# KangWelly/Assignment-for-AAE6102_GNSS-SDR

Hardware: AMD Instinct MI355X
Metric: correlator Msamples/s (acq+track), whole job (higher is better)
Workload: dtype int8 in; acquisition: f64 correlation + f64 fine search; tracking: f64

## Files before the change

assignment-for-aae6102_gnss-sdr_amd/abi.py:

```python
from __future__ import annotations

import ctypes as C
import os
import sys

MAX_SV = 64
MAX_TAPS = 32

OK, ENODATA, EIO, EARG, EDEVICE, EINDEX = 0, 1, 2, 3, 4, 5

FIELDS = ["P_i", "P_q", "E_i", "E_q", "L_i", "L_q", "PLLdiscri", "DLLdiscri", "codedelay",
          "remChip", "codeFreq", "carrierFreq", "remPhase", "remSample", "numSample",
          "delayValue", "absoluteSample", "codedelay2"]
NFIELDS = len(FIELDS)
OUT_DEVICE = 1
FIELDS_POS = ["P_i", "P_q", "E_i", "E_q", "L_i", "L_q", "carrError", "codeError", "codedelay",
              "remChip", "codeFreq", "carrFreq", "remCarrPhase", "absoluteSampleCodedelay",
              "numSample", "delayValue", "absoluteSample", "codedelay2"]

MC_TAPS = 25
MC_TAP_NAMES = ([f"E_{{}}{s}" for s in ["_060", "_055", "", "_045", "_040", "_035", "_030", "_025",
                                         "_020", "_015", "_010", "_005"]] + ["P_{}"] +
                [f"L_{{}}{s}" for s in ["005", "010", "015", "020", "025", "030", "035", "040", "045",
                                         "", "055", "060"]])
# ... 143 lines not shown
    "gnss_abi_version": (C.c_int, []),
    "gnss_strerror": (C.c_char_p, [C.c_int]),
    "gnss_ctx_create": (C.c_int, [C.c_int, C.POINTER(C.c_void_p)]),
    "gnss_ctx_create_multi": (C.c_int, [C.POINTER(C.c_int), C.c_int, C.POINTER(C.c_void_p)]),
    "gnss_ctx_members": (C.c_int, [C.c_void_p]),
    "gnss_ctx_drop_record": (C.c_int, [C.c_void_p, C.c_void_p]),
    "gnss_ctx_resident_records": (C.c_int, [C.c_void_p]),
    "gnss_device_count": (C.c_int, []),
    "gnss_ctx_destroy": (None, [C.c_void_p]),
    "gnss_last_error": (C.c_char_p, [C.c_void_p]),
    "gnss_last_timing": (C.c_int, [C.c_void_p, C.POINTER(GnssTiming)]),
    "gnss_ctx_set_profiling": (C.c_int, [C.c_void_p, C.c_int]),
    "gnss_ctx_set_acq_precision": (C.c_int, [C.c_void_p, C.c_int]),
    "gnss_ctx_set_window": (C.c_int, [C.c_void_p, C.c_uint64]),
    "gnss_ctx_set_option": (C.c_int, [C.c_void_p, C.c_int, C.c_int64]),
    "gnss_dev_alloc": (C.c_int, [C.c_void_p, C.c_uint64, C.POINTER(C.c_void_p)]),
    "gnss_dev_free": (C.c_int, [C.c_void_p, C.c_void_p]),
    "gnss_dev_upload": (C.c_int, [C.c_void_p, C.c_void_p, C.c_void_p, C.c_uint64]),
    "gnss_dev_download": (C.c_int, [C.c_void_p, C.c_void_p, C.c_void_p, C.c_uint64]),
    "gnss_acquisition": (C.c_int, [C.c_void_p, C.POINTER(GnssFile), C.POINTER(GnssSignal),
                                   C.POINTER(GnssAcq), C.POINTER(GnssAcquired),
                                   C.POINTER(GnssAcqDiag)]),
    "gnss_tracking_ct": (C.c_int, [C.c_void_p, C.POINTER(GnssFile), C.POINTER(GnssSignal),
                                   C.POINTER(GnssTrack), C.POINTER(GnssAcquired),
                                   C.POINTER(GnssTrackOut)]),
    "gnss_tracking_ct_pos": (C.c_int, [C.c_void_p, C.POINTER(GnssFile), C.POINTER(GnssSignal),
                                       C.POINTER(GnssTrack), C.POINTER(GnssAcquired), C.c_int32,
                                       C.POINTER(C.c_int32), C.POINTER(GnssTrackOut)]),
    "gnss_tracking_ct_mc": (C.c_int, [C.c_void_p, C.POINTER(GnssFile), C.POINTER(GnssSignal),
                                      C.POINTER(GnssTrack), C.POINTER(GnssAcquired), C.c_int32,
                                      C.c_int32, C.POINTER(GnssTrackOut)]),
    "gnss_tracking_ct_multicorr": (C.c_int, [C.c_void_p, C.POINTER(GnssFile), C.POINTER(GnssSignal),
                                             C.POINTER(GnssTrack), C.POINTER(GnssAcquired), C.c_int32,
                                             C.POINTER(GnssTrackOut)]),
    "gnss_navi_decode": (C.c_int, [C.POINTER(GnssAcquired), C.POINTER(C.c_double),
                                   C.POINTER(C.c_int64), C.c_int64, C.POINTER(GnssNavOut)]),
    "gnss_lnav_bits": (C.c_int, [C.c_int32, C.c_int32, C.c_void_p]),
    "gnss_ca_code": (C.c_int, [C.c_int, C.c_void_p]),
    "gnss_correlate_step": (C.c_int, [C.c_void_p, C.POINTER(GnssFile), C.POINTER(GnssSignal),
                                      C.c_int, C.c_int, C.c_double, C.c_double, C.c_double,
                                      C.c_double, C.c_int64, C.c_int, C.POINTER(C.c_double),
                                      C.POINTER(C.c_double), C.POINTER(C.c_int64)]),
    "gnss_synth_if_device": (C.c_int, [C.c_void_p, C.POINTER(GnssSynth), C.c_uint64, C.c_uint64,
                                       C.c_void_p]),
    "gnss_tracking_vt_run": (C.c_int, [C.c_void_p, C.POINTER(GnssFile), C.POINTER(GnssSignal),
                                       C.POINTER(GnssTrack), C.c_int32, C.c_int32, C.c_int32,
                                       C.POINTER(GnssVtChan), C.POINTER(C.c_double), C.POINTER(GnssVtOut)]),
    "gnss_tracking_vt_step": (C.c_int, [C.c_void_p, C.POINTER(GnssFile), C.POINTER(GnssSignal),
                                        C.POINTER(GnssTrack), C.c_int32, C.c_int32, C.POINTER(GnssVtChan),
                                        C.POINTER(C.c_double), C.POINTER(GnssVtOut)]),
    "gnss_vt_nco_step": (C.c_int, [C.POINTER(GnssSignal), C.POINTER(GnssTrack), C.c_int32,
                                   C.POINTER(GnssVtChan), C.c_double, C.c_double, C.c_double,
                                   C.POINTER(GnssVtOut)]),
    "gnss_vt_prepare": (C.c_int, [C.POINTER(GnssSignal), C.c_int32, C.POINTER(GnssVtChan), C.c_double,
                                  C.POINTER(C.c_int32), C.POINTER(C.c_int64)]),
    "gnss_sv_pos_vel": (C.c_int, [C.POINTER(GnssEphSv), C.c_double, C.POINTER(C.c_double),
                                  C.POINTER(C.c_double), C.POINTER(C.c_double), C.POINTER(C.c_double),
                                  C.POINTER(C.c_double)]),
    "gnss_geo": (C.c_int, [C.c_int, C.POINTER(C.c_double), C.POINTER(C.c_double)]),
    "gnss_vt_nav_init": (C.c_int, [C.POINTER(GnssVtNavCfg), C.POINTER(GnssSignal), C.c_int32, C.c_int32,
                                   C.POINTER(C.c_int32), C.POINTER(GnssEphSv), C.POINTER(C.c_double),
                                   C.POINTER(C.c_double), C.c_double, C.c_double, C.POINTER(C.c_double),
                                   C.POINTER(GnssVtNav)]),
    "gnss_vt_nav_predict": (C.c_int, [C.POINTER(GnssVtNav), C.c_int32, C.c_int64, C.POINTER(C.c_double),
                                      C.POINTER(C.c_double), C.POINTER(C.c_double)]),
    "gnss_vt_nav_update": (C.c_int, [C.POINTER(GnssVtNav), C.POINTER(C.c_double), C.POINTER(C.c_double),
                                     C.POINTER(C.c_double), C.POINTER(GnssVtNavSol)]),
    "gnss_tracking_vt": (C.c_int, [C.c_void_p, C.POINTER(GnssFile), C.POINTER(GnssSignal), C.POINTER(GnssTrack),
                                   C.c_int32, C.c_int32, C.POINTER(GnssVtChan), C.POINTER(GnssVtNav),
                                   C.POINTER(GnssVtOut), C.POINTER(GnssVtNavSol)]),
    "gnss_tracking_vt_mc_run": (C.c_int, [C.c_void_p, C.POINTER(GnssFile), C.POINTER(GnssSignal),
                                          C.POINTER(GnssTrack), C.c_int32, C.c_int32, C.c_int32,
                                          C.POINTER(GnssVtChan), C.POINTER(C.c_double), C.POINTER(GnssVtMcOut)]),
    "gnss_tracking_vt_mc": (C.c_int, [C.c_void_p, C.POINTER(GnssFile), C.POINTER(GnssSignal), C.POINTER(GnssTrack),
                                      C.c_int32, C.c_int32, C.POINTER(GnssVtChan), C.POINTER(GnssVtNav),
                                      C.POINTER(GnssVtMcOut), C.POINTER(GnssVtNavSol)]),
    "gnss_vt_mc_prepare": (C.c_int, [C.POINTER(GnssSignal), C.c_int32, C.POINTER(GnssVtChan), C.c_double,
                                     C.POINTER(C.c_double), C.POINTER(C.c_double), C.POINTER(C.c_int64)]),
    "gnss_vt_mc_nco_step": (C.c_int, [C.POINTER(GnssSignal), C.POINTER(GnssTrack), C.c_int32,
                                      C.POINTER(GnssVtChan), C.c_double, C.POINTER(C.c_double),
                                      C.POINTER(C.c_double), C.POINTER(GnssVtMcOut)]),
    "gnss_vt_mc_nav_update": (C.c_int, [C.POINTER(GnssVtNav), C.POINTER(C.c_double), C.POINTER(C.c_double),
                                        C.POINTER(C.c_double), C.POINTER(GnssVtNavSol)]),
}

LIB_PATH = os.path.join(os.path.dirname(os.path.abspath(__file__)), "lib", "libgnss_mi355x.so")
_lib = None
_torch_first = False
LOADED_PATH = None

(OPT_FORCE_SUB, OPT_NO_PERSIST, OPT_FORCE_VPB, OPT_ACQ_ROCFFT, OPT_FINE_ROCFFT, OPT_ACQ_BATCH, OPT_ACQ_FUSED,
 OPT_ACQ_RING, OPT_ACQ_PIPE, OPT_VT_BLOCKS, OPT_FORCE_PEER, OPT_VT_SPAN) = range(12)
MAX_DEVICES = 16


def require_torch():
    import torch
    if _lib is not None and not _torch_first:
        raise RuntimeError("import torch before the first gnss Context / abi.load() "
                           "(PyTorch-ROCm must bring up its HIP runtime first)")
    return torch


class GnssError(RuntimeError):
    def __init__(self, status, msg=""):
        self.status = status
        super().__init__(f"gnss status {status}: {msg}")


def load(path: str | None = None):
    global _lib
    if _lib is not None and path is None:
        return _lib
    p = path or os.environ.get("GNSS_LIB") or LIB_PATH
    if not os.path.exists(p):
        raise ImportError(f"{p} missing: the HIP extension is not built "
                          "(run `python -c 'import __graft_entry__ as g; g.build()'`)")
    global _torch_first
    if _lib is None:
        if "torch" not in sys.modules and os.environ.get("GNSS_NO_TORCH", "0") != "1":
            try:
                import torch
            except Exception:
                pass
        _torch_first = "torch" in sys.modules
    lib = C.CDLL(p)
    for name, (res, args) in PROTOTYPES.items():
        if p != LIB_PATH and not hasattr(lib, name):
            continue
        fn = getattr(lib, name)
        fn.restype = res
        fn.argtypes = args
    if path is None:
        global LOADED_PATH
        _lib = lib
        LOADED_PATH = os.path.abspath(p)
    return lib
```

assignment-for-aae6102_gnss-sdr_amd/csrc/gnss_api.cpp:

```cpp
#include <hip/hip_runtime.h>
#include <rocfft/rocfft.h>

#include <algorithm>
#include <chrono>
#include <cstdarg>
#include <cmath>
#include <cstdio>
#include <cstring>
#include <cstdlib>
#include <functional>
#include <thread>
#include <vector>
#include <fcntl.h>
#include <map>
#include <memory>
#include <mutex>
#include <string>
#include <tuple>
#include <unistd.h>
#include <vector>

#include "gnss_internal.h"
#include "group.h"
#include "vt_mc.h"

using namespace gnss;

struct gnss_ctx {
    int device = 0;
    hipStream_t stream = nullptr;
    hipStream_t stream2 = nullptr;
    hipEvent_t ev_cols[2] = {}, ev_rows[2] = {};
    std::string err;
    gnss_timing timing{};
    int profiling = 0;
    std::map<std::tuple<size_t, size_t, int, int>, rocfft_plan> plans;
    void* fft_work = nullptr;
    size_t fft_work_size = 0;
    std::map<std::string, std::pair<void*, size_t>> pool;
    std::map<std::string, std::pair<void*, size_t>> pinned;
    int64_t acq_tw_S = 0;
    int acq_tw_dbl = -1;
    int acq_fp64 = 1;
    uint64_t window = 0;
    int64_t opt[GNSS_OPT_COUNT] = {};
    std::vector<gnss_ctx*> members;
    bool member = false;
    int fail_chan = -1;
    gnss::group::ResidentCache<void*> resident;
};

static void release_resident(void* p)
{
    if (p) (void)hipFree(p);
}

static int drop_resident(gnss_ctx* ctx, const void* p, uint64_t n)
{
    int k = 0;
    for (gnss_ctx* m : ctx->members) {
        (void)hipSetDevice(m->device);
        if (m->stream) (void)hipStreamSynchronize(m->stream);
        if (!p) {
            k += (int)m->resident.m.size();
            m->resident.clear(release_resident);
        } else {
            k += m->resident.drop_overlapping(p, n, release_resident);
        }
    }
    (void)hipSetDevice(ctx->device);
    return k;
}

#ifndef GNSS_PROBE_BUILD
#define GNSS_PROBE_BUILD 0
#endif
static const char* probe_env(const char* name)
{
    return GNSS_PROBE_BUILD ? getenv(name) : nullptr;
}

namespace {
constexpr int kAcqPipeDefault = 2;
#ifndef GNSS_ACQ_FWD_SPLIT
#define GNSS_ACQ_FWD_SPLIT 1
#endif
constexpr bool kAcqFwdSplit = GNSS_ACQ_FWD_SPLIT;
constexpr int kAcqPairFront = 60;
constexpr int kVtSpan = 2000;
constexpr int kFineBatch = 16;

template <class T>
T* pinned_buffer(gnss_ctx* ctx, const char* key, size_t count, unsigned flags = hipHostMallocDefault)
{
    auto& e = ctx->pinned[key];
    const size_t want = std::max<size_t>(count * sizeof(T), 16);
    if (e.second < want) {
        if (e.first) (void)hipHostFree(e.first);
        e = {nullptr, 0};
        if (hipHostMalloc(&e.first, want, flags) != hipSuccess) return nullptr;
        e.second = want;
    }
    return static_cast<T*>(e.first);
}
}

namespace {

int fail(gnss_ctx* ctx, int code, const char* fmt, ...) __attribute__((format(printf, 3, 4)));
int fail(gnss_ctx* ctx, int code, const char* fmt, ...)
{
    char buf[512];
    va_list ap;
    va_start(ap, fmt);
    vsnprintf(buf, sizeof buf, fmt, ap);
    va_end(ap);
    if (ctx) ctx->err = buf;
    return code;
}

bool lane_rate_admitted(const gnss_signal* sg, double codeFreq_max)
{
    return sg->Fs > 0 && 8.0 * std::max(sg->codeFreqBasis * 1.01, codeFreq_max) / sg->Fs < 1.0;
}

int refuse_lane_rate(gnss_ctx* ctx, const gnss_signal* sg, double codeFreq_max)
{
    return fail(ctx, GNSS_EARG,
// ... 697 lines not shown
    }
    std::vector<int> ds(devices, devices + n);
    std::sort(ds.begin(), ds.end());
    ds.erase(std::unique(ds.begin(), ds.end()), ds.end());
    for (int a : ds)
        for (int b : ds) {
            int can = 0;
            if (a == b || hipDeviceCanAccessPeer(&can, a, b) != hipSuccess || !can) continue;
            if (hipSetDevice(a) == hipSuccess) (void)hipDeviceEnablePeerAccess(b, 0);
            (void)hipGetLastError();
        }
    (void)hipSetDevice(devices[0]);
    *out = g;
    return GNSS_OK;
}

int gnss_device_count(void)
{
    int n = 0;
    if (hipGetDeviceCount(&n) != hipSuccess) return 0;
    return n;
}

int gnss_ctx_members(const gnss_ctx* ctx)
{
    if (!ctx) return 0;
    return ctx->members.empty() ? 1 : (int)ctx->members.size();
}

void gnss_ctx_destroy(gnss_ctx* ctx)
{
    if (!ctx) return;
    for (gnss_ctx* m : ctx->members) gnss_ctx_destroy(m);
    ctx->members.clear();
    (void)hipSetDevice(ctx->device);
    if (ctx->stream) (void)hipStreamSynchronize(ctx->stream);
    ctx->resident.clear(release_resident);
    if (ctx->stream2) (void)hipStreamSynchronize(ctx->stream2);
    for (auto& kv : ctx->plans) rocfft_plan_destroy(kv.second);
    if (ctx->fft_work) (void)hipFree(ctx->fft_work);
    for (auto& kv : ctx->pool)
        if (kv.second.first) (void)hipFree(kv.second.first);
    for (auto& kv : ctx->pinned)
        if (kv.second.first) (void)hipHostFree(kv.second.first);
    for (int i = 0; i < 2; i++) {
        if (ctx->ev_cols[i]) (void)hipEventDestroy(ctx->ev_cols[i]);
        if (ctx->ev_rows[i]) (void)hipEventDestroy(ctx->ev_rows[i]);
    }
    if (ctx->stream2) (void)hipStreamDestroy(ctx->stream2);
    if (ctx->stream) (void)hipStreamDestroy(ctx->stream);
    delete ctx;
}

const char* gnss_last_error(const gnss_ctx* ctx) { return ctx ? ctx->err.c_str() : "no context"; }

int gnss_last_timing(const gnss_ctx* ctx, gnss_timing* out)
{
    if (!ctx || !out) return GNSS_EARG;
    *out = ctx->timing;
    return GNSS_OK;
}

int gnss_ctx_set_profiling(gnss_ctx* ctx, int enable)
{
    if (!ctx) return GNSS_EARG;
    ctx->profiling = enable;
    for (gnss_ctx* m : ctx->members) m->profiling = enable;
    return GNSS_OK;
}

int gnss_ctx_set_window(gnss_ctx* ctx, uint64_t bytes)
{
    if (!ctx) return GNSS_EARG;
    ctx->window = bytes;
    for (gnss_ctx* m : ctx->members) m->window = bytes;
    return GNSS_OK;
}

int gnss_ctx_set_option(gnss_ctx* ctx, int key, int64_t value)
{
    if (!ctx || key < 0 || key >= GNSS_OPT_COUNT) return GNSS_EARG;
    if (key == GNSS_OPT_VT_BLOCKS && (value < 0 || value > GNSS_VT_MAX_BLOCKS))
        return fail(ctx, GNSS_EARG, "GNSS_OPT_VT_BLOCKS outside 0..%d", GNSS_VT_MAX_BLOCKS);
    if (key == GNSS_OPT_VT_SPAN && (value < 0 || value > kVtSpan))
        return fail(ctx, GNSS_EARG, "GNSS_OPT_VT_SPAN outside 0..%d", kVtSpan);
    ctx->opt[key] = value;
    for (gnss_ctx* m : ctx->members) m->opt[key] = value;
    return GNSS_OK;
}

int gnss_ctx_set_acq_precision(gnss_ctx* ctx, int fp64)
{
    if (!ctx || (fp64 != 0 && fp64 != 1)) return GNSS_EARG;
    ctx->acq_fp64 = fp64;
    for (gnss_ctx* m : ctx->members) m->acq_fp64 = fp64;
    return GNSS_OK;
}

int gnss_dev_alloc(gnss_ctx* ctx, uint64_t nbytes, void** dev_ptr)
{
    if (!ctx || !dev_ptr) return GNSS_EARG;
    HIP_TRY(hipSetDevice(ctx->device));
    HIP_TRY(hipMalloc(dev_ptr, nbytes ? nbytes : 16));
    return GNSS_OK;
}

int gnss_ctx_drop_record(gnss_ctx* ctx, const void* dev_ptr)
{
    if (!ctx) return GNSS_EARG;
    drop_resident(ctx, dev_ptr, 0);
    return GNSS_OK;
}

int gnss_ctx_resident_records(const gnss_ctx* ctx)
{
    if (!ctx) return 0;
    int k = 0;
    for (const gnss_ctx* m : ctx->members) k += (int)m->resident.m.size();
    return k;
}

int gnss_dev_free(gnss_ctx* ctx, void* p)
{
    if (!ctx) return GNSS_EARG;
    drop_resident(ctx, p, 0);
    HIP_TRY(hipSetDevice(ctx->device));
    HIP_TRY(hipFree(p));
    return GNSS_OK;
}

int gnss_dev_upload(gnss_ctx* ctx, void* dst, const void* src, uint64_t n)
{
    if (!ctx) return GNSS_EARG;
    drop_resident(ctx, dst, n);
    HIP_TRY(hipSetDevice(ctx->device));
    HIP_TRY(hipMemcpyAsync(dst, src, n, hipMemcpyHostToDevice, ctx->stream));
    HIP_TRY(hipStreamSynchronize(ctx->stream));
    return GNSS_OK;
}

int gnss_dev_download(gnss_ctx* ctx, void* dst, const void* src, uint64_t n)
{
    if (!ctx) return GNSS_EARG;
    HIP_TRY(hipSetDevice(ctx->device));
    HIP_TRY(hipMemcpyAsync(dst, src, n, hipMemcpyDeviceToHost, ctx->stream));
    HIP_TRY(hipStreamSynchronize(ctx->stream));
    return GNSS_OK;
}

int gnss_acquisition(gnss_ctx* ctx, const gnss_file* file, const gnss_signal* sg,
                     const gnss_acq* acq, gnss_acquired* out, gnss_acq_diag* diag)
{
    if (!ctx || !file || !sg || !acq || !out) return GNSS_EARG;
    if (!ctx->members.empty()) return group_acquisition(ctx, file, sg, acq, out, diag);
    memset(out, 0, sizeof(*out));
    if (diag) memset(diag, 0, sizeof(*diag));
    ctx->timing = gnss_timing{};
    HIP_TRY(hipSetDevice(ctx->device));
    const int prec = file->dataPrecision, dtyp = file->dataType;
    if ((prec != 1 && prec != 2) || (dtyp != 1 && dtyp != 2))
        return fail(ctx, GNSS_EARG, "dataPrecision must be 1 (int8) or 2 (int16), dataType 1 (I) or 2 (I/Q)");
    if (prec == 2 && dtyp == 1)
        return fail(ctx, GNSS_EINDEX, "int16 real record: rawsignal has Sample*datalen/2 samples (MATLAB index error)");
    const int64_t bps = (int64_t)prec * dtyp;
    const bool iq8 = prec == 1 && dtyp == 2;
    const int64_t S = sg->Sample;
// ... 329 lines not shown
        }
        const int64_t c0 = (S - cd + 1 + (file->skip + N1 + 18) * S) * bps;
        const int64_t a1 = (S - cd + 1 + file->skip * S) * bps + (int64_t)((N1 + 18) * S * 1.01 + 64) * bps;
        hi = std::max(hi, std::max(c0 + (int64_t)(n10 * 10 * S * 1.01 + 4096) * bps, a1));
        hiA = std::max(hiA, a1);
    }
    P.file_len = file_length(file);
    if (P.file_len < 0) return fail(ctx, GNSS_EIO, "cannot open IF record");
    IfWindow w;
    lo &= ~(int64_t)31;
    const bool seg = ctx->window > 0 && !file->dev_data && !pos && !gv && prec == 1 && dtyp == 2 && n10 > 0 &&
                     (uint64_t)(hi - lo) > ctx->window;
    int st;
    if (seg) {
        if ((uint64_t)(hiA - lo) > ctx->window || ctx->window < (uint64_t)(12 * S * bps * 1.01 + 8192))
            return fail(ctx, GNSS_EARG, "window budget below the 1-ms phases' span");
        HIP_TRY(w.own.alloc(ctx->window + 64));
        w.ptr = w.own.as<int8_t>();
        w.base = lo;
        w.len = std::min<int64_t>(hiA, P.file_len) - lo;
        if ((st = stage_into(ctx, file, w.base, w.base + w.len, w.own.as<int8_t>()))) return st;
    } else if ((st = stage_window(ctx, file, lo, hi, w))) {
        return st;
    }
    const int8_t* iq_dev = w.ptr;
    P.buf_base = w.base;
    P.buf_len = w.len;
    DevBuf d_conv, d_pref, d_pscr;
    {
        const int64_t s0 = std::max<int64_t>(lo, w.base);
        const int64_t s1 = std::min<int64_t>(hi, w.base + w.len);
        const int8_t* src = w.ptr + (s0 - w.base);
        if (prec == 1 && dtyp == 1) {
            const int64_t n = std::max<int64_t>(s1 - s0, 0);
            HIP_TRY(d_conv.alloc(ctx, "trk.d_conv", (size_t)(2 * n + 64)));
            HIP_TRY(launch_real8_to_iq8(src, n, d_conv.as<int8_t>(), ctx->stream));
            iq_dev = d_conv.as<int8_t>();
            P.buf_base = 2 * s0;
            P.buf_len = 2 * n;
        } else if (prec == 2) {
            iq_dev = src;
            P.buf_base = s0;
            P.buf_len = std::max<int64_t>(s1 - s0, 0);
            const int64_t ng = P.buf_len / 32;
            HIP_TRY(d_pref.alloc(ctx, "trk.d_pref", 2 * sizeof(long long) * (size_t)(ng + 1)));
            const size_t scr = prefix16_scratch_bytes(ng);
            HIP_TRY(d_pscr.alloc(ctx, "trk.d_pscr", scr));
            long long* pi = d_pref.as<long long>();
            HIP_TRY(launch_prefix16(reinterpret_cast<const short*>(src), ng, pi, pi + ng + 1, d_pscr.p, scr,
                                    ctx->stream));
            P.pref_i = pi;
            P.pref_q = pi + ng + 1;
            P.stage16 = reinterpret_cast<const short*>(iq_dev - P.buf_base);
        }
    }

    const double cps_max = 1.1 * sg->codeFreqBasis / sg->Fs;
    auto sub_ok = [&](int sub) { return 8.0 * sub * cps_max < 1.0 && (sub == 1 || !P.exact_div); };
    auto sub_for = [&](int pdi) {
        int sub = pdi >= 10 ? 3 : 1;
        while (sub > 1 && !sub_ok(sub)) sub--;
        if ((P.fmt == 1 || ntaps == 25) && sub != 3) sub = 1;
        return sub;
    };
    int sub1 = sub_for(1), sub10 = sub_for(10);
    if (const char* fs = probe_env("GNSS_FORCE_SUB10")) {
        const int v = atoi(fs);
        if (v >= 1 && v <= 4 && sub_ok(v) && P.fmt == 0 && ntaps != 25) sub10 = v;
    }
    if (const char* fs = probe_env("GNSS_FORCE_SUB1")) {
        const int v = atoi(fs);
        if (v >= 1 && v <= 4 && sub_ok(v) && P.fmt == 0 && ntaps != 25) sub1 = v;
    }
    if (const int v = (int)ctx->opt[GNSS_OPT_FORCE_SUB]) {
        if (v >= 1 && v <= 4 && sub_ok(v) && ((P.fmt == 0 && ntaps != 25) || v == 1 || v == 3)) sub1 = sub10 = v;
    }
    auto bpc_for = [&](int pdi, int sub) {
        const double groups = (S * pdi * 1.01 + 64) / 8.0 + 2;
        return (int)std::ceil(groups / ((double)kTrkThreads * sub));
    };
    int cus = 0;
    HIP_TRY(hipDeviceGetAttribute(&cus, hipDeviceAttributeMultiprocessorCount, ctx->device));
    P.qcap_dmax = cps_max;
    auto qcap_ok = [&](int sub) {
        return !GNSS_QCAP || P.ntaps <= 3 ||
               max_taps_in_lane(P.taps, P.tap_post, P.ntaps, 8 * sub, cps_max) <= kQcapMax;
    };
    auto vpb_for = [&](int pdi, int sub) {
        if (ctx->opt[GNSS_OPT_NO_PERSIST] || P.fmt != 0 || wide_taps || bpc_for(pdi, sub) > run_bpc_cap(P.ntaps) ||
            !qcap_ok(sub))
            return 0;
        const int bpc = bpc_for(pdi, sub);
        int v0 = 1;
        if (ctx->opt[GNSS_OPT_FORCE_VPB] > 0) v0 = (int)std::min<int64_t>(ctx->opt[GNSS_OPT_FORCE_VPB], kMaxVpb);
        const int occ1 = std::min(track_run_blocks_per_cu(P, sub, false), 4);
        if (v0 == 1 && occ1 >= 1 && (int64_t)nch * bpc <= (int64_t)occ1 * cus) return 1;
        const int occv = std::min(track_run_blocks_per_cu(P, sub, true), 4);
        if (occv < 1) return 0;
        for (int v = std::max(v0, 2); v <= kMaxVpb; v++)
            if ((int64_t)nch * ((bpc + v - 1) / v) <= (int64_t)occv * cus) return v;
        return 0;
    };
    const int vpb1 = vpb_for(1, sub1), vpb10 = vpb_for(10, sub10);
    bool persist1 = vpb1 > 0, persist10 = vpb10 > 0;
    if (const char* pr = probe_env("GNSS_PROBE")) P.probe = atoi(pr);
    const int bpc1 = bpc_for(1, sub1), bpc10 = bpc_for(10, sub10);
    if (bpc10 > kMaxBpc) return fail(ctx, GNSS_EARG, "Sample too large for the step geometry");

    std::vector<TrkChan> ch0((size_t)nch);
    std::vector<unsigned> cab((size_t)nch * 32);
    for (int i = 0; i < nch; i++) {
        const int c = chans[i];
        TrkChan& t = ch0[i];
        memset(&t, 0, sizeof(t));
        t.codeFreq = sg->codeFreqBasis;
        t.carrierFreqBasis = acq->fineFreq[c];
        t.carrierFreq = acq->fineFreq[c];
        t.codedelay0 = acq->codedelay[c];
        t.pos = (S - acq->codedelay[c] + 1 + file->skip * S) * bps;
        t.snrIndex = 1;
        t.sv1 = c + 1;
        t.prn = acq->sv[c];
        t.n1_target = N1;
        if (pos) {
            t.pos = (int64_t)(((double)S - acq->codedelay[c] + 1 + (double)file->skip * sg->Fs * sg->ms) * bps);
            t.codedelay0 = S - acq->codedelay[c] + 1;
            t.sv1 = 1;
            t.n1_target = pos_n1(c);
            t.countinx = pos->countinx ? pos->countinx[c] : 0;
        }
        if (gv) t.pos = (S - acq->codedelay[c] - 1 + file->skip * S) * bps;
        if (acq->sv[c] < 1 || acq->sv[c] > 51) return fail(ctx, GNSS_EARG, "bad PRN");
        ca_bits(acq->sv[c], &cab[(size_t)i * 32]);
    }
    DevBuf d_chan, d_snap, d_desc, d_ca, d_part, d_arrive, d_rec, d_taps, d_cn1, d_cn10, d_dv, d_pi;
    HIP_TRY(d_chan.alloc(ctx, "trk.d_chan", sizeof(TrkChan) * nch));
    HIP_TRY(d_snap.alloc(ctx, "trk.d_snap", sizeof(TrkChan) * nch));
    HIP_TRY(d_desc.alloc(ctx, "trk.d_desc", sizeof(StepDesc) * nch));
    HIP_TRY(d_ca.alloc(ctx, "trk.d_ca", sizeof(unsigned) * cab.size()));
    HIP_TRY(d_part.alloc(ctx, "trk.d_part", sizeof(double) * (size_t)nch * kMaxBpc * 2 * ntaps));
    const size_t arrive_bytes = sizeof(unsigned) * kArrivePerChan * kArriveStride * nch;
    HIP_TRY(d_arrive.alloc(ctx, "trk.d_arrive", arrive_bytes));
    HIP_TRY(d_rec.alloc(ctx, "trk.d_rec", sizeof(double) * (size_t)nch * P.rec_cap * GNSS_NFIELDS));
    if (out->taps) HIP_TRY(d_taps.alloc(ctx, "trk.d_taps", sizeof(double) * (size_t)nch * P.rec_cap * 2 * ntaps));
    HIP_TRY(d_cn1.alloc(ctx, "trk.d_cn1", sizeof(double) * (size_t)nch * P.cn0_cap));
    HIP_TRY(d_cn10.alloc(ctx, "trk.d_cn10", sizeof(double) * (size_t)nch * P.cn0_cap));
    HIP_TRY(d_dv.alloc(ctx, "trk.d_dv", sizeof(int64_t) * (size_t)nch * (P.rec_cap + 1)));
    HIP_TRY(d_pi.alloc(ctx, "trk.d_pi", sizeof(double) * (size_t)nch * N1));
    HIP_TRY(hipMemcpyAsync(d_chan.p, ch0.data(), sizeof(TrkChan) * nch, hipMemcpyHostToDevice, ctx->stream));
    HIP_TRY(hipMemcpyAsync(d_ca.p, cab.data(), sizeof(unsigned) * cab.size(), hipMemcpyHostToDevice, ctx->stream));
    HIP_TRY(hipMemsetAsync(d_arrive.p, 0, arrive_bytes, ctx->stream));
    HIP_TRY(hipMemsetAsync(d_cn1.p, 0, d_cn1.n, ctx->stream));
    HIP_TRY(hipMemsetAsync(d_cn10.p, 0, d_cn10.n, ctx->stream));
    HIP_TRY(hipMemsetAsync(d_dv.p, 0, d_dv.n, ctx->stream));
    HIP_TRY(hipMemsetAsync(d_rec.p, 0, d_rec.n, ctx->stream));

    TrkBuffers B{};
    B.iq = iq_dev;
    B.chan = d_chan.as<TrkChan>();
    B.snap = d_snap.as<TrkChan>();
    B.desc = d_desc.as<StepDesc>();
    B.ca_bits = d_ca.as<unsigned>();
    B.partial = d_part.as<double>();
    B.arrive = d_arrive.as<unsigned>();
    B.rec = d_rec.as<double>();
    B.taps_rec = out->taps ? d_taps.as<double>() : nullptr;
    B.cn0_1 = d_cn1.as<double>();
    B.cn0_10 = d_cn10.as<double>();
    B.dvpre = d_dv.as<int64_t>();
    B.p_i_1ms = d_pi.as<double>();
    B.n1 = N1;

    DevBuf d_stamps;
    const char* stamp_path = probe_env("GNSS_STAMPS");
    if (stamp_path) {
        HIP_TRY(d_stamps.alloc(ctx, "trk.d_stamps", sizeof(unsigned long long) * ((size_t)kStampSlots * (8 + 3 * kMaxBpc) + 1)));
        HIP_TRY(hipMemsetAsync(d_stamps.p, 0, d_stamps.n, ctx->stream));
        B.stamps = d_stamps.as<unsigned long long>();
    }

    DevBuf d_pgran, d_err;
    if (persist1 || persist10) {
        HIP_TRY(d_pgran.alloc(ctx, "trk.d_pgran", sizeof(unsigned long long) * 2 * (size_t)nch * gran_per_chan(ntaps)));
        HIP_TRY(d_err.alloc(ctx, "trk.d_err", 16));
        HIP_TRY(hipMemsetAsync(d_pgran.p, 0, d_pgran.n, ctx->stream));
        HIP_TRY(hipMemsetAsync(d_err.p, 0, 16, ctx->stream));
        B.pgran = d_pgran.as<unsigned long long>();
        B.run_err = d_err.as<unsigned>();
    }
// ... 253 lines not shown
        const double* src;
        int64_t stride;
        if (f < nrf) {
            dst = out->rec + ((int64_t)c * GNSS_NFIELDS + f) * ML;
            src = rec + (size_t)i * P.rec_cap * GNSS_NFIELDS + f;
            stride = GNSS_NFIELDS;
        } else {
            const int tq = f - nrf, sidx = tq / 2, iq = tq % 2;
            dst = out->taps + (((int64_t)c * 2 + iq) * ntaps + sidx) * ML;
            src = tp + (size_t)i * P.rec_cap * 2 * ntaps + tq;
            stride = 2 * ntaps;
        }
        for (int64_t k = 0; k < n1; k++) dst[k] = src[k * stride];
        for (int64_t q = 0; q < n10; q++) {
            const double v = src[(n1 + q) * stride];
            for (int r = 0; r < 10; r++) dst[n1 + 10 * q + r] = v;
        }
        for (int64_t k = n1 + 10 * n10; k < ML; k++) dst[k] = 0;
    });
    if (hp) fprintf(stderr, "hostprof expanded %.3f ms\n", hms());
    if (gv && out->rec) {
        for (int c = 0; c < nsv; c++) {
            double* cdr = out->rec + ((int64_t)c * GNSS_NFIELDS + GNSS_F_codedelay) * ML;
            double sum = 0;
            for (int64_t k = 0; k < N1; k++) {
                const int r = (int)(k % nsv);
                if (r <= c) sum += out->rec[((int64_t)r * GNSS_NFIELDS + GNSS_F_delayValue) * ML + k / nsv];
                cdr[k] = (double)acq->codedelay[c] + sum;
            }
        }
    }
    rows = std::max(rows, n10 / 20);
    out->cn0_rows = rows;
    if (out->CN0_Eph) {
        for (int i = 0; i < nch; i++) {
            const int c = chans[i];
            const int cx = chh[i].countinx;
            const int r1 = pos ? rows : std::max(N1, N1 + cx) / 20, r10 = n10 / 20;
            for (int r = 0; r < out->cn0_cap; r++) {
                double v = 0;
                if (r < r10) v = cn10[(size_t)i * P.cn0_cap + r];
                else if (r < r1) v = cn1[(size_t)i * P.cn0_cap + r];
                out->CN0_Eph[(int64_t)r * nsv + c] = v;
            }
        }
    }
    return GNSS_OK;
}

int gnss_tracking_ct(gnss_ctx* ctx, const gnss_file* file, const gnss_signal* sg, const gnss_track* tr,
                     const gnss_acquired* acq, gnss_track_out* out)
{
    if (ctx && !ctx->members.empty()) return group_tracking(ctx, file, sg, tr, acq, out, nullptr);
    return tracking_impl(ctx, file, sg, tr, acq, out, nullptr);
}

int gnss_tracking_ct_pos(gnss_ctx* ctx, const gnss_file* file, const gnss_signal* sg, const gnss_track* tr,
                         const gnss_acquired* acq, int32_t ctPOS, const int32_t* countinx, gnss_track_out* out)
{
    const PosCfg pc{ctPOS, countinx, 0};
    if (ctx && !ctx->members.empty()) return group_tracking(ctx, file, sg, tr, acq, out, &pc);
    return tracking_impl(ctx, file, sg, tr, acq, out, &pc);
}

int gnss_tracking_ct_multicorr(gnss_ctx* ctx, const gnss_file* file, const gnss_signal* sg,
                               const gnss_track* tr, const gnss_acquired* acq, int32_t datalength,
                               gnss_track_out* out)
{
    const GivenCfg g{datalength};
    return tracking_impl(ctx, file, sg, tr, acq, out, nullptr, &g);
}

int gnss_tracking_ct_mc(gnss_ctx* ctx, const gnss_file* file, const gnss_signal* sg, const gnss_track* tr,
                        const gnss_acquired* acq, int32_t msPosCT, int32_t pdi, gnss_track_out* out)
{
    if (!ctx) return GNSS_EARG;
    if (pdi != 1 && pdi != 10) return fail(ctx, GNSS_EARG, "multicorrelator: pdi must be 1 or 10");
    if (msPosCT < pdi) return fail(ctx, GNSS_EARG, "multicorrelator: msPosCT/pdi must be >= 1");
    const PosCfg pc{msPosCT / pdi, nullptr, pdi};
    if (!ctx->members.empty()) return group_tracking(ctx, file, sg, tr, acq, out, &pc);
    return tracking_impl(ctx, file, sg, tr, acq, out, &pc);
}

int gnss_correlate_step(gnss_ctx* ctx, const gnss_file* file, const gnss_signal* sg, int prn, int pdi,
                        double remChip, double codeFreq, double carrierFreq, double remPhase,
                        int64_t pos_bytes, int n_taps, const double* taps, double* sums_out,
                        int64_t* numSample_out)
{
    if (!ctx || !file || !sg || !taps || !sums_out || (n_taps != 3 && n_taps != 11) || prn < 1 || prn > 51)
        return GNSS_EARG;
    if (pdi != 1 && pdi != 10) return GNSS_EARG;
    if (!lane_rate_admitted(sg, codeFreq)) return refuse_lane_rate(ctx, sg, codeFreq);
    HIP_TRY(hipSetDevice(ctx->device));
    const int64_t S = sg->Sample;
    TrkParams P{};
    P.Fs = sg->Fs;
    P.codeFreqBasis = sg->codeFreqBasis;
    P.ms = sg->ms;
    P.codelength = sg->codelength;
    P.S = (double)S;
    P.dataBytesPerSample = 2;
    P.bps = 2;
    P.fmt = 0;
    P.inv_Fs = 1.0 / sg->Fs;
    P.exact_div = fast_div_exact(sg->Fs, (int64_t)(S * 10 * 1.02) + 64) ? 0 : 1;
    P.ntaps = n_taps;
    P.iE = 0; P.iP = n_taps / 2; P.iL = n_taps - 1;
    for (int s = 0; s < n_taps; s++) P.taps[s] = taps[s];
    P.nsv = P.nch = 1;
    P.rec_cap = 1;
    P.cn0_cap = 1;
    P.file_len = file_length(file);
    IfWindow w;
    int st = stage_window(ctx, file, pos_bytes, pos_bytes + (int64_t)(2.1 * S * pdi) + 64, w);
    if (st) return st;
    P.buf_base = w.base;
    P.buf_len = w.len;
    TrkChan c{};
    c.remChip = remChip;
    c.codeFreq = codeFreq;
    c.carrierFreq = carrierFreq;
    c.remPhase = remPhase;
    c.pos = pos_bytes;
    c.n1_target = 1 << 30;
    c.sv1 = 1;
    c.prn = prn;
    unsigned cab[32];
    ca_bits(prn, cab);
    int sub = 1;
    if (const int v = (int)ctx->opt[GNSS_OPT_FORCE_SUB]) {
        if (v >= 2 && v <= 4 && !P.exact_div && 8.0 * v * codeFreq / sg->Fs < 1.0) sub = v;
    }
    const int bpc = (int)std::ceil(((S * pdi * 1.01 + 64) / 8.0 + 2) / ((double)kTrkThreads * sub));
    DevBuf d_chan, d_desc, d_ca, d_part, d_arrive, d_sums;
    HIP_TRY(d_chan.alloc(sizeof(TrkChan)));
    HIP_TRY(d_desc.alloc(sizeof(StepDesc)));
    HIP_TRY(d_ca.alloc(sizeof(cab)));
    HIP_TRY(d_part.alloc(sizeof(double) * kMaxBpc * 2 * n_taps));
    HIP_TRY(d_arrive.alloc(sizeof(unsigned) * kArrivePerChan * kArriveStride));
    HIP_TRY(d_sums.alloc(sizeof(double) * 2 * n_taps));
    HIP_TRY(hipMemcpyAsync(d_chan.p, &c, sizeof c, hipMemcpyHostToDevice, ctx->stream));
    HIP_TRY(hipMemcpyAsync(d_ca.p, cab, sizeof cab, hipMemcpyHostToDevice, ctx->stream));
    HIP_TRY(hipMemsetAsync(d_arrive.p, 0, sizeof(unsigned) * kArrivePerChan * kArriveStride, ctx->stream));
    TrkBuffers B{};
    B.iq = w.ptr;
    B.chan = d_chan.as<TrkChan>();
    B.desc = d_desc.as<StepDesc>();
    B.ca_bits = d_ca.as<unsigned>();
    B.partial = d_part.as<double>();
    B.arrive = d_arrive.as<unsigned>();
    B.dbg_sums = d_sums.as<double>();
    DevBuf d_args;
    HIP_TRY(d_args.alloc(sizeof(TrkParams) + sizeof(TrkBuffers)));
    HIP_TRY(hipMemcpyAsync(d_args.p, &P, sizeof(TrkParams), hipMemcpyHostToDevice, ctx->stream));
    HIP_TRY(hipMemcpyAsync(static_cast<char*>(d_args.p) + sizeof(TrkParams), &B, sizeof(TrkBuffers),
                           hipMemcpyHostToDevice, ctx->stream));
    const TrkDev TD{d_args.as<TrkParams>(),
                    reinterpret_cast<const TrkBuffers*>(static_cast<char*>(d_args.p) + sizeof(TrkParams))};

    HIP_TRY(launch_track_prepare(P, B, TD, pdi, 0, ctx->stream));
    HIP_TRY(launch_track_step(P, B, TD, bpc, sub, ctx->stream));
    HIP_TRY(hipMemcpyAsync(sums_out, d_sums.p, sizeof(double) * 2 * n_taps, hipMemcpyDeviceToHost, ctx->stream));
    HIP_TRY(hipMemcpyAsync(&c, d_chan.p, sizeof c, hipMemcpyDeviceToHost, ctx->stream));
    HIP_TRY(hipStreamSynchronize(ctx->stream));
    if (c.status) return fail(ctx, c.status, "correlate step failed");
    if (numSample_out) {
        const double cps = codeFreq / sg->Fs;
        *numSample_out = (int64_t)round((sg->codelength * pdi - remChip) / cps);
    }
    return GNSS_OK;
}

}

void gnss::ca_chips(int prn, float* out) { generate_ca(prn, out); }

extern "C" {

int gnss_tracking_vt_run(gnss_ctx* ctx, const gnss_file* file, const gnss_signal* sg, const gnss_track* tr,
                         int32_t pdi, int32_t n, int32_t nsteps, gnss_vt_chan* chans, const double* codeFreq_new,
                         gnss_vt_out* out)
{
    if (!ctx || !file || !sg || !tr || !chans || !codeFreq_new || !out || n < 1 || n > GNSS_MAX_SV || pdi < 1 ||
        nsteps < 1 || !(sg->Fs > 0) || !(sg->codeFreqBasis > 0))
        return fail(ctx, GNSS_EARG, "bad arguments");
    ctx->err.clear();
    ctx->timing = gnss_timing{};
    HIP_TRY(hipSetDevice(ctx->device));
    const int prec = file->dataPrecision, dtyp = file->dataType;
    if (!((prec == 1 && (dtyp == 1 || dtyp == 2)) || (prec == 2 && dtyp == 2)))
        return fail(ctx, GNSS_EARG, "vector tracking: int8 I/Q, int8 real or int16 I/Q records");
    const int bps = prec * dtyp;
    const int64_t flen = file_length(file);
    if (flen < 0) return fail(ctx, GNSS_EIO, "cannot open IF record");
    double cf_min = 1e300;
    for (int i = 0; i < n; i++) {
        if (chans[i].prn < 1 || chans[i].prn > 51) return fail(ctx, GNSS_EARG, "bad PRN");
        if (chans[i].file_ptr < 0 || chans[i].file_ptr % bps) return fail(ctx, GNSS_EARG, "file_ptr");
        if (chans[i].index_int < 0 || chans[i].index_int > 19 || chans[i].snrIndex < 1)
            return fail(ctx, GNSS_EARG, "C/N0 state (index_int 0..19, snrIndex >= 1)");
        cf_min = std::min(cf_min, chans[i].codeFreq);
    }
    for (int64_t k = 0; k < (int64_t)nsteps * n; k++) cf_min = std::min(cf_min, codeFreq_new[k]);
    if (!(cf_min > 0)) return fail(ctx, GNSS_EARG, "code frequencies must be positive");
    const double nmax = std::ceil((sg->codelength * pdi + 2.0) / (cf_min / sg->Fs)) + 2;
    int64_t lo = INT64_MAX, hi = 0;
    for (int i = 0; i < n; i++) {
        lo = std::min(lo, chans[i].file_ptr);
        hi = std::max(hi, chans[i].file_ptr + (int64_t)(nsteps * nmax) * bps);
    }
    IfWindow w;
    int st = stage_window(ctx, file, lo, std::min(hi, flen), w);
    if (st) return st;
    std::vector<unsigned> cab((size_t)n * 32);
    for (int i = 0; i < n; i++) ca_bits(chans[i].prn, &cab[(size_t)i * 32]);
// ... 770 lines not shown
```

assignment-for-aae6102_gnss-sdr_amd/csrc/gnss_internal.h:

```cpp
#pragma once

#include <hip/hip_runtime.h>
#include <stdint.h>

#include "../../include/gnss_mi355x.h"

#define GNSS_HD __host__ __device__ __forceinline__

namespace gnss {

struct Colon {
    double a, d, c;
    int64_t n;
};

GNSS_HD Colon colon_make(double a, double d, double b)
{
    Colon r{a, d, b, -1};
    if (!(a - a == 0) || !(d - d == 0) || !(b - b == 0)) return r;
    if (d == 0 || (a < b && d < 0) || (b < a && d > 0)) return r;
    double tol = 2.0 * 2.220446049250313e-16 * fmax(fabs(a), fabs(b));
    double sig = d > 0 ? 1.0 : -1.0;
    double n;
    if (a == floor(a) && d == 1) {
// ... 125 lines not shown
    const int n = (int)q & 3;
    const double a = (n & 1) ? c : s, b = (n & 1) ? s : c;
    *sn = (n & 2) ? -a : a;
    *cs = ((n + 1) & 2) ? -b : b;
}


typedef unsigned u32x4 __attribute__((ext_vector_type(4)));
constexpr int kBufRsrcWord3 = 0x00020000;
constexpr int kPolSc1 = 16;

__device__ __forceinline__ void publish16(__amdgpu_buffer_rsrc_t r, int unit, double v, unsigned tag)
{
    const unsigned long long w = (unsigned long long)__double_as_longlong(v);
    const u32x4 g = {(unsigned)w, tag, (unsigned)(w >> 32), tag};
    __builtin_amdgcn_raw_buffer_store_b128(g, r, unit * 16, 0, kPolSc1);
}
__device__ __forceinline__ u32x4 load16(__amdgpu_buffer_rsrc_t r, int unit)
{
    return __builtin_amdgcn_raw_buffer_load_b128(r, unit * 16, 0, kPolSc1);
}
constexpr int kPolSys = 17;
__device__ __forceinline__ void publish16_sys(__amdgpu_buffer_rsrc_t r, int unit, double v, unsigned tag)
{
    const unsigned long long w = (unsigned long long)__double_as_longlong(v);
    const u32x4 g = {(unsigned)w, tag, (unsigned)(w >> 32), tag};
    __builtin_amdgcn_raw_buffer_store_b128(g, r, unit * 16, 0, kPolSys);
}
__device__ __forceinline__ u32x4 load16_sys(__amdgpu_buffer_rsrc_t r, int unit)
{
    return __builtin_amdgcn_raw_buffer_load_b128(r, unit * 16, 0, kPolSys);
}
__device__ __forceinline__ double value16(u32x4 g)
{
    return __longlong_as_double((long long)(((unsigned long long)g.z << 32) | g.x));
}

struct TrkChan {
    double remChip, remPhase, remSample;
    double carrier_outputLast, PLLdiscriLast, code_outputLast, DLLdiscriLast;
    double codeFreq, carrierFreqBasis, carrierFreq;
    double Zk[20];
    int64_t numSample;
    int64_t pos;
    int64_t Index;
    int64_t nstep;
    int64_t slot;
    int64_t n1_target;
    int64_t codedelay0;
    int32_t index_int, snrIndex;
    int32_t sv1;
    int32_t prn;
    int32_t status;
    int32_t countinx;
};

struct TrkParams {
    double Fs, codeFreqBasis, ms, codelength;
    double S;
    double tau1code, tau2code, tau1carr, tau2carr;
    double dataBytesPerSample;
    double inv_Fs;
    int32_t exact_div;
    int64_t buf_base;
    int64_t buf_len;
    int64_t file_len;
    int32_t ntaps, iE, iP, iL;
    int32_t nsv;
    int32_t nch;
    int32_t rec_cap;
    int32_t cn0_cap;
    int32_t probe;
    int32_t bps, fmt;
    const long long* pref_i;
    const long long* pref_q;
    const short* stage16;
    double taps[GNSS_MAX_TAPS];
    double qcap_dmax;
    double dll_r, dll_t1, dll_t10, pll_r, pll_t1, pll_t10;
    int32_t conv;
    int32_t chip_off;
    int32_t given;
    double tap_post[GNSS_MAX_TAPS];
};

constexpr int kLaneMax = 32;

struct StepDesc {
    int64_t n, delayValue, A, g_first, g_last, Index;
    double remSample, d, inv_d, f, phi0, dhi, dlo, remChip_next, remPhase_next;
    double mu_r, mu_i;
    double phi[kLaneMax];
    double2 rcs[kLaneMax];
    double tap_a[GNSS_MAX_TAPS], tap_c[GNSS_MAX_TAPS];
    double rc0;
    int32_t pdi, phaseC;
    int32_t bad;
    int32_t bad_tap;
};

struct TrkBuffers {
    const int8_t* iq;
    TrkChan* chan;
    TrkChan* snap;
    StepDesc* desc;
    const unsigned* ca_bits;
    double* partial;
    unsigned int* arrive;
    double* rec;
    double* taps_rec;
    double* cn0_1;
    double* cn0_10;
    int64_t* dvpre;
    double* p_i_1ms;
    double* dbg_sums;
    unsigned long long* stamps;
    unsigned long long* pgran;
    unsigned* run_err;
    int32_t n1;
};

struct TrkDev {
    const TrkParams* p;
    const TrkBuffers* b;
};

hipError_t launch_track_step(const TrkParams& p, const TrkBuffers& b, const TrkDev& d,
                             int blocks_per_chan, int sub, hipStream_t s);
hipError_t launch_track_run(const TrkParams& p, const TrkBuffers& b, const TrkDev& d,
                            int blocks_per_chan, int vblocks_per_block, int sub, int nsteps, unsigned tag0,
                            hipStream_t s);
int track_run_blocks_per_cu(const TrkParams& p, int sub, bool vblocks = false);
hipError_t launch_track_prepare(const TrkParams& p, const TrkBuffers& b, const TrkDev& d, int pdi,
                                int phaseC, hipStream_t s);
hipError_t launch_track_snapshot(const TrkParams& p, const TrkBuffers& b, const TrkDev& d, hipStream_t s);
hipError_t launch_track_bitedge(const TrkParams& p, const TrkBuffers& b, const TrkDev& d, hipStream_t s);
hipError_t launch_track_phase_c_init(const TrkParams& p, const TrkBuffers& b, const TrkDev& d,
                                     int64_t skip, hipStream_t s);
hipError_t launch_track_expand(const double* src, int64_t rec_cap, int stride, int nf, int nch,
                               const int64_t* job, double* dst, int64_t ML, int64_t n10, int ntaps,
                               hipStream_t s);

#ifndef GNSS_PROBE_BUILD
#define GNSS_PROBE_BUILD 0
#endif
constexpr bool kProbe = GNSS_PROBE_BUILD != 0;
#ifndef GNSS_XCHG_SLEEP
#define GNSS_XCHG_SLEEP 0
#endif
#ifndef GNSS_XCD_LOCAL
#define GNSS_XCD_LOCAL 0
#endif

constexpr int kTrkThreads = 256;
constexpr int kArriveStride = 64;
constexpr int kArrivePerChan = 9;
constexpr int kStampSlots = 2200;
constexpr int kMaxBpc = 1024;
constexpr int kMaxBpcRun = 256;
constexpr int run_bpc_cap(int ntaps) { return ntaps > 3 ? 192 : kMaxBpcRun; }
constexpr int kMaxVpb = 16;
#ifndef GNSS_QCAP
#define GNSS_QCAP 0
#endif
constexpr double kTapSpan = 30.0;
constexpr int kQcapMax = 8;

inline int max_taps_in_lane(const double* taps, const double* post, int n, int M, double dmax)
{
    const double w = (M - 1) * dmax + 1e-9;
    int best = 0;
    for (int a = 0; a < n; a++) {
        const double x = taps[a] + (post ? post[a] : 0.0);
        int c = 0;
        for (int b = 0; b < n; b++) {
            double f = (taps[b] + (post ? post[b] : 0.0)) - x;
            f -= floor(f);
            if (f < w || f > 1.0 - 1e-9) c++;
        }
        best = c > best ? c : best;
    }
    return best;
}
constexpr int kDeferSlots = 4;
constexpr int gran_region_b(int ntaps) { return ntaps > 3 ? 2 * kMaxBpcRun * 6 : 0; }
constexpr int gran_slot_b(int ntaps) { return 2 * ntaps * kMaxBpcRun; }
constexpr int gran_per_chan(int ntaps)
{
    return ntaps > 3 ? gran_region_b(ntaps) + kDeferSlots * gran_slot_b(ntaps) : 2 * kMaxBpcRun * 2 * ntaps;
}
constexpr int kDescWords = (int)(sizeof(StepDesc) / 4);

struct AcqPeak {
    double peak;
    int32_t fbin;
    int32_t cp;
    double snr;
    double peak2;
};

hipError_t launch_acq_wipe(const int8_t* iq, const double2* xs, int64_t S, int datalen, int nbins, double IF,
                           double freqMin, double freqStep, double Fs, float2* out, hipStream_t s);
hipError_t launch_acq_code(const float* ca, const int32_t* prn_slot, int nprn, int64_t S,
                           double codeFreqBasis, double Fs, float2* out, hipStream_t s);
hipError_t launch_acq_mul(const float2* code_spec, const float2* sig_spec, int nprn, int nsig,
                          int64_t S, float2* out, hipStream_t s);
hipError_t launch_acq_power(const float2* y, int nprn, int nbins, int datalen, int64_t S,
                            int first_ms, float* corr, hipStream_t s);
hipError_t launch_acq_wipe(const int8_t* iq, const double2* xs, int64_t S, int datalen, int nbins, double IF,
                           double freqMin, double freqStep, double Fs, double2* out, hipStream_t s);
hipError_t launch_acq_code(const float* ca, const int32_t* prn_slot, int nprn, int64_t S,
                           double codeFreqBasis, double Fs, double2* out, hipStream_t s);
hipError_t launch_acq_mul(const double2* code_spec, const double2* sig_spec, int nprn, int nsig,
                          int64_t S, double2* out, hipStream_t s);
hipError_t launch_acq_power(const double2* y, int nprn, int nbins, int datalen, int64_t S,
                            int first_ms, double* corr, hipStream_t s);
hipError_t launch_acq_peak(const float* corr, int nprn, int nbins, int64_t S, int cshift,
                           int perm, AcqPeak* out, void* scratch, hipStream_t s);
hipError_t launch_acq_peak(const double* corr, int nprn, int nbins, int64_t S, int cshift,
                           int perm, AcqPeak* out, void* scratch, hipStream_t s);

bool acq_fft_supported(int64_t S);
template <class V>
hipError_t launch_acq_fft_forward(const int8_t* iq, const double2* xs, int64_t S, int datalen, int nbins, double IF,
                                  double freqMin, double freqStep, double Fs, const float* ca,
                                  int nprn, double codeFreqBasis, const V* tw_row,
                                  const V* tw_col, V* B, V* X, hipStream_t s, int bin0 = 0, int nbc = -1,
                                  bool codes = true);
constexpr int kAcqCols = 1, kAcqRows = 2;
hipError_t launch_acq_fft_correlate(const float2* C, const float2* X, int64_t S, int datalen,
                                    int nbins, int nprn, int first_pair, int npair,
                                    const float2* tw_row, const float2* tw_col, float2* A,
                                    float* corr, hipStream_t s, int parts = kAcqCols | kAcqRows);
hipError_t launch_acq_fft_correlate(const double2* C, const double2* X, int64_t S, int datalen,
                                    int nbins, int nprn, int first_pair, int npair,
                                    const double2* tw_row, const double2* tw_col, double2* A,
                                    double* corr, hipStream_t s, int parts = kAcqCols | kAcqRows);
hipError_t launch_acq_fft_pair(const double2* C, const double2* X, int64_t S, int datalen, int nbins, int nprn,
                               int cols_first, int cols_n, double2* Acols, int rows_first, int rows_n,
                               const double2* Arows, const double2* tw_row, const double2* tw_col, double* corr,
                               int front, hipStream_t s);
size_t acq_fused_sync_bytes();
size_t acq_fused_err_offset();
size_t acq_fused_ring_bytes(int64_t S);
hipError_t launch_acq_fft_correlate_fused(const double2* C, const double2* X, int64_t S, int datalen, int nbins,
                                          int nprn, int nslot, const double2* tw_row, const double2* tw_col,
                                          double2* ring, void* sync, double* corr, hipStream_t s);
bool fine_fft_supported(int64_t S, int L);
size_t fine_fft_scratch_bytes(int64_t S, int L, int datalen, int nsv);
hipError_t launch_fine_fft_tables(int64_t S, int L, int datalen, void* scratch, hipStream_t s);
hipError_t launch_fine_fft_argmax(const int8_t* iq, const double2* xs, int64_t S, int L, int datalen,
                                  const int32_t* cd, int nsv, const float* ca, double Fs, double codeFreqBasis,
                                  double codelength, int shifted, void* scratch, int64_t* kbest, hipStream_t s);
hipError_t launch_fine_build(const int8_t* iq, const double2* xs, int64_t S, int L, const int32_t* codedelay,
                             const float* ca, int nsv, double Fs, double codeFreqBasis,
                             double codelength, int64_t N, double2* out, hipStream_t s);
hipError_t launch_fine_argmax(const double2* F, int nsv, int64_t N, int shifted, void* scratch,
                              int64_t* kbest, hipStream_t s);

size_t acq_scratch_bytes(int nprn, int nsv);

hipError_t launch_stage_cpx(const int8_t* src, int prec, int type, int64_t nsamp, double2* out,
                            unsigned long long* sums, hipStream_t s);
hipError_t launch_real8_to_iq8(const int8_t* src, int64_t n, int8_t* dst, hipStream_t s);
size_t prefix16_scratch_bytes(int64_t ngroups);
// ... 268 lines not shown
```

assignment-for-aae6102_gnss-sdr_amd/csrc/track.hip:

```cpp
#include "gnss_internal.h"

namespace gnss {

namespace {

constexpr int kStampRow = 8 + 3 * kMaxBpc;

__device__ __forceinline__ unsigned long long* stamp_row(const TrkBuffers& b)
{
    const unsigned long long cnt = __hip_atomic_load(b.stamps + (size_t)kStampSlots * kStampRow,
                                                     __ATOMIC_RELAXED, __HIP_MEMORY_SCOPE_AGENT);
    return b.stamps + (cnt % kStampSlots) * kStampRow;
}

__device__ __forceinline__ void stamp_max(unsigned long long* row, int k, unsigned long long v)
{
    row[k] = v;
}

__device__ __forceinline__ int uni(int v) { return __builtin_amdgcn_readfirstlane(v); }
__device__ __forceinline__ int64_t uni(int64_t v)
{
    const int lo = __builtin_amdgcn_readfirstlane((int)v);
    const int hi = __builtin_amdgcn_readfirstlane((int)(v >> 32));
    return (int64_t)(((uint64_t)(uint32_t)hi << 32) | (uint32_t)lo);
}
__device__ __forceinline__ double uni(double v) { return __longlong_as_double(uni((int64_t)__double_as_longlong(v))); }

typedef int i32x4 __attribute__((ext_vector_type(4)));
typedef __attribute__((address_space(1))) const i32x4 g_i32x4;
typedef __attribute__((address_space(1))) double g_dbl;
typedef __attribute__((address_space(1))) long long g_i64;
typedef __attribute__((address_space(1))) unsigned g_u32;
typedef __attribute__((address_space(1))) unsigned long long g_u64;
typedef __attribute__((address_space(1))) const StepDesc g_desc;
typedef __attribute__((address_space(1))) const TrkChan g_chan;
typedef __attribute__((address_space(1))) const unsigned g_cu32;

__device__ __forceinline__ int4 ld_g16(const int8_t* p)
{
    const i32x4 v = *(g_i32x4*)p;
    return make_int4(v.x, v.y, v.z, v.w);
}

__device__ __forceinline__ double ld_sc1(const double* ptr)
{
    return __hip_atomic_load((g_dbl*)ptr, __ATOMIC_RELAXED, __HIP_MEMORY_SCOPE_AGENT);
}

__device__ __forceinline__ void st_sc1(double* ptr, double v)
{
    __hip_atomic_store((g_dbl*)ptr, v, __ATOMIC_RELAXED, __HIP_MEMORY_SCOPE_AGENT);
}

__device__ __forceinline__ unsigned atomic_add_agent(unsigned* p, unsigned v)
{
    return __hip_atomic_fetch_add((g_u32*)p, v, __ATOMIC_RELAXED, __HIP_MEMORY_SCOPE_AGENT);
}

__device__ __forceinline__ void store_agent(unsigned* p, unsigned v)
{
    __hip_atomic_store((g_u32*)p, v, __ATOMIC_RELAXED, __HIP_MEMORY_SCOPE_AGENT);
}

__device__ __forceinline__ void store_agent(unsigned long long* p, unsigned long long v)
{
    __hip_atomic_store((g_u64*)p, v, __ATOMIC_RELAXED, __HIP_MEMORY_SCOPE_AGENT);
}

__device__ __forceinline__ unsigned long long load_agent(const unsigned long long* p)
{
    return __hip_atomic_load((g_u64*)p, __ATOMIC_RELAXED, __HIP_MEMORY_SCOPE_AGENT);
}

struct TailK {
    double Fs, inv_Fs, codelength, S, codeFreqBasis, ms;
    double dll_r, dll_t1, dll_t10, pll_r, pll_t1, pll_t10, tau1code, tau1carr, qcap_dmax;
    int32_t exact_div, conv, given, chip_off, ntaps, iE, iP, iL, bps;
    int64_t file_len, buf_base, buf_len;
    const double* taps;
    const double* tap_post;
    static constexpr int fmt = 0;
    static constexpr const long long* pref_i = nullptr;
// ... 454 lines not shown
        index_int = 0;
        snrIndex += 1;
    }
    g->remChip = o.remChip;
    g->remPhase = o.remPhase;
    g->remSample = o.remSample;
    g->carrier_outputLast = u.carrier_output;
    g->PLLdiscriLast = u.PLLdiscri;
    g->code_outputLast = u.code_output;
    g->DLLdiscriLast = u.DLLdiscri;
    g->codeFreq = u.codeFreq;
    g->carrierFreq = u.carrierFreq;
    g->numSample = o.n;
    g->pos = c.pos + p.bps * o.n;
    g->Index = c.Index + (o.phaseC ? 10 : 1);
    g->nstep = c.nstep + 1;
    g->slot = c.slot + 1;
    g->index_int = index_int;
    g->snrIndex = snrIndex;
}
__device__ __noinline__ void write_state(const TrkParams& p, const TrkBuffers& b, int ch, TrkChan* g, const TrkChan& c, const StepOut& o, const LoopUpd& u, const double* s, bool io)
{
    write_state_i(p, b, ch, g, c, o, u, s, io);
}

__device__ __forceinline__ void update_state_inplace(const TrkParams& p, const TrkBuffers& b, int ch,
                                                     TrkChan& c, const StepOut& o, const LoopUpd& u,
                                                     const double* s, bool io)
{
    const double P_i = s[2 * p.iP], P_q = s[2 * p.iP + 1];
    int index_int = c.index_int + 1;
    int snrIndex = c.snrIndex;
    c.Zk[index_int - 1] = P_i * P_i + P_q * P_q;
    if (index_int % 20 == 0) {
        if (io) {
            double Z[20];
#pragma unroll
            for (int k = 0; k < 20; k++) Z[k] = c.Zk[k];
            const double cn = cn0_estimate(Z, 1 * p.ms * o.pdi);
            g_dbl* cn0 = (g_dbl*)(o.phaseC ? b.cn0_10 : b.cn0_1);
            if (snrIndex <= p.cn0_cap) cn0[(int64_t)ch * p.cn0_cap + snrIndex - 1] = cn;
        }
        index_int = 0;
        snrIndex += 1;
    }
    const int64_t pos = c.pos, Index = c.Index, nstep = c.nstep, slot = c.slot;
    c.remChip = o.remChip;
    c.remPhase = o.remPhase;
    c.remSample = o.remSample;
    c.carrier_outputLast = u.carrier_output;
    c.PLLdiscriLast = u.PLLdiscri;
    c.code_outputLast = u.code_output;
    c.DLLdiscriLast = u.DLLdiscri;
    c.codeFreq = u.codeFreq;
    c.carrierFreq = u.carrierFreq;
    c.numSample = o.n;
    c.pos = pos + p.bps * o.n;
    c.Index = Index + (o.phaseC ? 10 : 1);
    c.nstep = nstep + 1;
    c.slot = slot + 1;
    c.index_int = index_int;
    c.snrIndex = snrIndex;
}


}

__device__ __forceinline__ double2 ld_rcs(const StepDesc* d, int m) { return d->rcs[m]; }
__device__ __forceinline__ double2 ld_rcs(g_desc* d, int m)
{
    typedef __attribute__((address_space(1))) const double g_cdbl;
    g_cdbl* q = (g_cdbl*)&d->rcs[m];
    return make_double2(q[0], q[1]);
}

template <int SUB> struct RegRaw {
    const int4 (&r)[SUB];
    __device__ __forceinline__ int4 get(int j) const { return r[j]; }
};
struct LdsRaw {
    const int4* p;
    __device__ __forceinline__ int4 get(int j) const { return p[j * kTrkThreads]; }
};

#ifndef GNSS_CORR_PROBE
#define GNSS_CORR_PROBE 0
#endif
#ifndef GNSS_IO_DR_WAVE
#define GNSS_IO_DR_WAVE 2
#endif
#ifndef GNSS_SWEEP_IO_ALL
#define GNSS_SWEEP_IO_ALL 0
#endif
#ifndef GNSS_FLUSH_PROBE
#define GNSS_FLUSH_PROBE 0
#endif

__device__ __forceinline__ unsigned ca_bits_ext(unsigned cabits, int lane)
{
    const unsigned w0 = __shfl(cabits, 0, 64), w1 = __shfl(cabits, 1, 64), w2 = __shfl(cabits, 2, 64);
    if (lane == 31) return cabits | ((w0 & 1u) << 31);
    if (lane == 32) return (w0 >> 1) | (w1 << 31);
    if (lane == 33) return (w1 >> 1) | (w2 << 31);
    return cabits;
}

#ifndef GNSS_SWP
#define GNSS_SWP 0
#endif
#ifndef GNSS_REGCAP
#define GNSS_REGCAP 0
#endif
#ifndef GNSS_PHI_REG
#define GNSS_PHI_REG 0
#endif
#ifndef GNSS_TAPWIN
#define GNSS_TAPWIN 1
#endif
template <int NT, int SUB, bool DIVIDE, bool RELOAD, int FMT, class Desc, class Raw>
__device__ __forceinline__ void lane_correlate(const TrkParams& p, const Desc* dp, const Raw& raw,
                                               int64_t ks, unsigned cabits, double2* myslot,
                                               const double2* zero, double (&oI)[NT], double (&oQ)[NT],
                                               const double* posts = nullptr)
{
    constexpr int M = 8 * SUB;
    constexpr int T = kTrkThreads;
    constexpr bool QC = RELOAD && (GNSS_QCAP == 2 || (GNSS_QCAP && NT > 3));
    if constexpr ((GNSS_CORR_PROBE & 8) != 0) {
#pragma unroll
        for (int s = 0; s < NT; s++) { oI[s] = 0.0; oQ[s] = 0.0; }
        return;
    }
    const int64_t n = uni(dp->n);
    const double d = uni(dp->d), inv_d = uni(dp->inv_d);
    const double f = uni(dp->f), phi0 = uni(dp->phi0);
    const double Fs = p.Fs, rFs = p.inv_Fs;

    const int ksi = (int)ks, ni = (int)n;
    const int lo = ksi < 0 ? (-ksi < M ? -ksi : M) : 0;
    const int hi = ni - ksi < M ? (ni - ksi > 0 ? ni - ksi : 0) : M;

    const int kfi0 = ksi + lo;
    const int kfi = kfi0 < 0 ? 0 : (kfi0 > ni - 1 ? ni - 1 : kfi0);
    const int64_t kf = kfi;
    int cap[NT];
    unsigned neg0 = 0u, neg1 = 0u;
    constexpr bool TW = GNSS_TAPWIN && RELOAD && (GNSS_CORR_PROBE & 66) == 0;
    if constexpr (TW) {
        const int nn = ni - 1;
        const bool mid = 2 * kfi == nn, lower = kfi <= nn / 2;
        const double KD = (double)kfi * d, NKD = (double)(nn - kfi) * d;
        const double kend = lower ? KD : -NKD;
        const double dk = (double)(kfi - ksi);
        int c0i[NT];
        int cmin = 0x7fffffff;
        bool exact = mid;
#pragma unroll
        for (int s = 0; s < NT; s++) {
            const double a = lds_at(dp->tap_a, s), c = lds_at(dp->tap_c, s);
            const double t0 = ((lower ? a : c) + kend) + lds_at(posts, s);
            const double c0 = ceil(t0);
            const double R = __builtin_fma(c0 - t0, inv_d, dk);
            exact = exact || fabs(R - rint(R)) < 1e-6;
            const int pb = (int)floor(R) + 1;
            cap[s] = (pb < M ? pb : M) - 1;
            c0i[s] = (int)c0;
        }
        if (exact) {
#pragma unroll
            for (int s = 0; s < NT; s++) {
                const double a = lds_at(dp->tap_a, s), c = lds_at(dp->tap_c, s);
                const double post = lds_at(posts, s);
                const double t0 = (mid ? (a + c) / 2 : lower ? a + KD : c - NKD) + post;
                const double c0 = ceil(t0);
                const double R = dk + (c0 - t0) * inv_d;
                const double rr = rint(R);
                int pb = (int)floor(R) + 1;
                if (fabs(R - rr) < 1e-6) {
                    const int ms = (int)rr;
                    pb = ms;
                    const int64_t kx = ks + ms;
                    if (ms >= 0 && ms < M && kx >= 0 && kx <= n - 1)
                        pb = ceil(colon_elem(Colon{a, d, c, (int64_t)nn}, kx) + post) > c0 ? ms : ms + 1;
                }
                cap[s] = (pb < M ? pb : M) - 1;
                c0i[s] = (int)c0;
            }
        }
#pragma unroll
        for (int s = 0; s < NT; s++) {
            if constexpr ((GNSS_CORR_PROBE & 32) != 0) cap[s] = M - 1 - s;
            cmin = c0i[s] < cmin ? c0i[s] : cmin;
        }
        const unsigned ib = ca_index32(cmin + p.chip_off);
        const unsigned wlo = __shfl(cabits, (int)(ib >> 5), 64), whi = __shfl(cabits, (int)(ib >> 5) + 1, 64);
        const unsigned long long W = (((unsigned long long)whi << 32) | wlo) >> (ib & 31);
#pragma unroll
        for (int s = 0; s < NT; s++) {
            const int o = c0i[s] - cmin;
            neg0 |= (unsigned)((W >> o) & 1ull) << s;
            neg1 |= (unsigned)((W >> (o + 1)) & 1ull) << s;
        }
    }
#pragma unroll
    for (int s = 0; s < (TW ? 0 : NT); s++) {
        if constexpr ((GNSS_CORR_PROBE & 2) != 0) {
            cap[s] = M - 1 - s;
            neg0 |= (cabits & 1u) << s;
            continue;
        }
        if constexpr ((GNSS_CORR_PROBE & 64) != 0) {
            cap[s] = (int)((ks + 5 * s) & 31) - 4;
            neg0 |= (cabits & 1u) << s;
            continue;
        }
        const Colon col{uni(dp->tap_a[s]), d, uni(dp->tap_c[s]), n - 1};
        const double post = p.tap_post[s];
        const double t0 = colon_elem(col, kf) + post;
        const double c0 = ceil(t0);
        const double R = (double)(int)(kf - ks) + (c0 - t0) * inv_d;
        const double rr = rint(R);
        int pb = (int)floor(R) + 1;
        if (fabs(R - rr) < 1e-6) {
            const int ms = (int)rr;
            pb = ms;
            const int64_t kx = ks + ms;
            if (ms >= 0 && ms < M && kx >= 0 && kx <= n - 1)
                pb = ceil(colon_elem(col, kx) + post) > c0 ? ms : ms + 1;
        }
        cap[s] = (pb < M ? pb : M) - 1;
        if constexpr ((GNSS_CORR_PROBE & 32) != 0) cap[s] = M - 1 - s;
        const unsigned i0 = ca_index32((int)c0 + p.chip_off);
        const unsigned i1 = i0 == 1022u ? 0u : i0 + 1u;
        const unsigned w0 = __shfl(cabits, (int)(i0 >> 5), 64);
        const unsigned w1 = __shfl(cabits, (int)(i1 >> 5), 64);
        neg0 |= ((w0 >> (i0 & 31)) & 1u) << s;
        neg1 |= ((w1 >> (i1 & 31)) & 1u) << s;
    }

    const double kb = (double)(int)ks;
    const double Wb = wave_at<DIVIDE>(kb, f, phi0, Fs, rFs);
    double sb, cb;
    if constexpr ((GNSS_CORR_PROBE & 1) != 0) {
        sb = Wb * 1e-9;
        cb = 1.0;
    } else {
        sincos_wave(Wb, &sb, &cb);
    }

    double run_r = 0.0, run_i = 0.0;
    double pre_r[QC ? 1 : NT], pre_i[QC ? 1 : NT];
    if constexpr (!QC) {
#pragma unroll
        for (int s = 0; s < NT; s++) { pre_r[s] = 0.0; pre_i[s] = 0.0; }
    }
    unsigned cmask = 0u;
    if constexpr (QC) {
#pragma unroll
        for (int s = 0; s < NT; s++)
            if (cap[s] >= 0 && cap[s] < M - 1) cmask |= 1u << cap[s];
    }

    double mu_r = 0.0, mu_i = 0.0;
    if constexpr (FMT == 1) {
        mu_r = uni(dp->mu_r);
        mu_i = uni(dp->mu_i);
    }

    constexpr bool RC = GNSS_REGCAP && !QC && NT <= 3;
    double dhi_l = 0.0, dlo_l = 0.0;
    if constexpr (GNSS_PHI_REG) {
        dhi_l = uni(dp->dhi);
        dlo_l = uni(dp->dlo);
    }
    double Wpipe = 0.0;
    if constexpr (GNSS_SWP) Wpipe = wave_at<DIVIDE>(kb + 1.0, f, phi0, Fs, rFs);
    auto subgroup = [&](const int j) {
        constexpr int NW = FMT == 1 ? 8 : 4;
        unsigned wd[NW];
        bool part = lo > 8 * j || hi < 8 * j + 8;
        if constexpr (FMT == 1) {
            const int4 ra = raw.get(2 * j), rb = raw.get(2 * j + 1);
            wd[0] = (unsigned)ra.x; wd[1] = (unsigned)ra.y; wd[2] = (unsigned)ra.z; wd[3] = (unsigned)ra.w;
            wd[4] = (unsigned)rb.x; wd[5] = (unsigned)rb.y; wd[6] = (unsigned)rb.z; wd[7] = (unsigned)rb.w;
        } else {
            const int4 rj = raw.get(j);
            wd[0] = (unsigned)rj.x; wd[1] = (unsigned)rj.y; wd[2] = (unsigned)rj.z; wd[3] = (unsigned)rj.w;
            if (part) {
#pragma unroll
                for (int q = 0; q < 4; q++) {
                    const int m0 = 8 * j + 2 * q;
                    const unsigned k0 = (m0 >= lo && m0 < hi) ? 0x0000FFFFu : 0u;
                    const unsigned k1 = (m0 + 1 >= lo && m0 + 1 < hi) ? 0xFFFF0000u : 0u;
                    wd[q] &= k0 | k1;
                }
            }
        }
        const double kbj = kb + (double)(8 * j);
#pragma unroll
        for (int mm = 0; mm < 8; mm++) {
            const int m = 8 * j + mm;
            double xr, xi;
            if constexpr (FMT == 1) {
                const unsigned word = wd[mm];
                xr = (double)(short)(word & 0xFFFFu) - mu_r;
                xi = (double)(short)(word >> 16) - mu_i;
                if (part && !(m >= lo && m < hi)) { xr = 0.0; xi = 0.0; }
            } else {
                const unsigned word = wd[mm >> 1];
                const int sh = (mm & 1) * 16;
                xr = (double)(int8_t)((word >> sh) & 0xFF);
                xi = (double)(int8_t)((word >> (sh + 8)) & 0xFF);
            }
            if constexpr ((GNSS_CORR_PROBE & 4) != 0) {
                const double2 rcs = ld_rcs(dp, m);
                run_r = __builtin_fma(xr, rcs.x, run_r);
                run_r = __builtin_fma(-xi, rcs.y, run_r);
                run_i = __builtin_fma(xr, rcs.y, run_i);
                run_i = __builtin_fma(xi, rcs.x, run_i);
            } else if (m > 0) {
                double W;
                if constexpr (GNSS_SWP) {
                    W = Wpipe;
                    if (m + 1 < M) Wpipe = wave_at<DIVIDE>(kbj + (double)(mm + 1), f, phi0, Fs, rFs);
                } else {
                    W = wave_at<DIVIDE>(kbj + (double)mm, f, phi0, Fs, rFs);
                }
                double phm;
                if constexpr (GNSS_PHI_REG) phm = (double)m * dhi_l + (double)m * dlo_l;
                else phm = dp->phi[m];
                const double eta = (W - Wb) - phm;
                const double2 rcs = ld_rcs(dp, m);
                const double rc = __builtin_fma(-eta, rcs.y, rcs.x);
                const double rs = __builtin_fma(eta, rcs.x, rcs.y);
                run_r = __builtin_fma(xr, rc, run_r);
                run_r = __builtin_fma(-xi, rs, run_r);
                run_i = __builtin_fma(xr, rs, run_i);
                run_i = __builtin_fma(xi, rc, run_i);
            } else {
                run_r += xr;
                run_i += xi;
            }
            if constexpr (QC) {
                if ((cmask >> m) & 1u)
                    myslot[__builtin_popcount(cmask & ((1u << m) - 1u)) * T] = make_double2(run_r, run_i);
            } else if constexpr (RC) {
#pragma unroll
                for (int s = 0; s < NT; s++) {
                    const bool at = cap[s] == m;
                    pre_r[s] = at ? run_r : pre_r[s];
                    pre_i[s] = at ? run_i : pre_i[s];
                }
            } else {
                myslot[mm * T] = make_double2(run_r, run_i);
            }
            if constexpr (GNSS_SWP == 2) __builtin_amdgcn_sched_barrier(0);
        }
        if constexpr (!QC && !RC) {
#pragma unroll
            for (int s = 0; s < NT; s++) {
                const unsigned idx = (unsigned)(cap[s] - 8 * j);
                const double2 v = *(idx < 8u ? myslot + idx * T : zero);
                pre_r[s] += v.x;
                pre_i[s] += v.y;
            }
        }
    };
#ifndef GNSS_UNROLL_TAPS
#define GNSS_UNROLL_TAPS 0
#endif
    if constexpr (RELOAD && ((NT > 3 && !GNSS_UNROLL_TAPS) || (RC && GNSS_REGCAP == 2))) {
#pragma unroll 1
        for (int j = 0; j < SUB; j++) subgroup(j);
    } else if constexpr (RELOAD) {
#pragma unroll
        for (int j = 0; j < SUB; j++) subgroup(j);
    } else {
#pragma unroll
        for (int j = 0; j < SUB; j++) subgroup(j);
    }

#pragma unroll
    for (int s = 0; s < NT; s++) {
        const double a0 = ((neg0 >> s) & 1u) ? -1.0 : 1.0;
        const double v1 = ((neg1 >> s) & 1u) ? -1.0 : 1.0;
        const double dv = a0 - v1;
        double pr, pi;
        if constexpr (QC) {
            const int cs = cap[s];
            const int q = __builtin_popcount(cmask & ((1u << (cs > 0 ? cs : 0)) - 1u));
            const double2 v = myslot[(q < 8 ? q : 7) * T];
            pr = (cs < 0 ? 0.0 : cs == M - 1 ? run_r : v.x) + 0.0;
            pi = (cs < 0 ? 0.0 : cs == M - 1 ? run_i : v.y) + 0.0;
        } else {
            pr = pre_r[s];
            pi = pre_i[s];
        }
        const double ur = __builtin_fma(dv, pr, v1 * run_r);
        const double ui = __builtin_fma(dv, pi, v1 * run_i);
        oI[s] = __builtin_fma(cb, ui, sb * ur);
        oQ[s] = __builtin_fma(cb, ur, -(sb * ui));
    }
}

template <int CTRL>
__device__ __forceinline__ double dpp_f64(double v)
{
    const long long b = __double_as_longlong(v);
    const int lo = __builtin_amdgcn_mov_dpp((int)b, CTRL, 0xF, 0xF, false);
    const int hi = __builtin_amdgcn_mov_dpp((int)(b >> 32), CTRL, 0xF, 0xF, false);
    return __longlong_as_double(((long long)hi << 32) | (unsigned)lo);
}

__device__ __forceinline__ void lds_barrier()
{
    __builtin_amdgcn_s_waitcnt(0xc07f);
    __builtin_amdgcn_s_barrier();
}

#ifndef GNSS_RED_ONEPASS
#define GNSS_RED_ONEPASS 11
#endif
template <int NT> constexpr int red_taps() { return NT > 3 ? (NT + 1) / 2 : NT; }
template <int NT> constexpr int run_red_taps() { return NT <= GNSS_RED_ONEPASS ? NT : red_taps<NT>(); }
template <int HT> constexpr int red_words() { return 2 * HT * (kTrkThreads + 32); }

#ifndef GNSS_RED
#define GNSS_RED 0
#endif
__device__ __forceinline__ double readlane_f64(double v, int l)
{
    const long long b = __double_as_longlong(v);
    const int lo = __builtin_amdgcn_readlane((int)b, l);
    const int hi = __builtin_amdgcn_readlane((int)(b >> 32), l);
    return __longlong_as_double(((long long)hi << 32) | (unsigned)lo);
}

template <int CTRL, int ROWS>
__device__ __forceinline__ double dpp_f64_rows(double v)
{
    const long long b = __double_as_longlong(v);
    const int lo = __builtin_amdgcn_update_dpp(0, (int)b, CTRL, ROWS, 0xF, false);
    const int hi = __builtin_amdgcn_update_dpp(0, (int)(b >> 32), CTRL, ROWS, 0xF, false);
    return __longlong_as_double(((long long)hi << 32) | (unsigned)lo);
}

__device__ __forceinline__ double wave_sum(double a)
{
    if constexpr (GNSS_RED == 2) {
        a += dpp_f64<0xB1>(a);
        a += dpp_f64<0x4E>(a);
        a += dpp_f64<0x141>(a);
        a += dpp_f64<0x140>(a);
        a += dpp_f64_rows<0x142, 0xA>(a);
// ... 73 lines not shown
        }
        if (t >= 0 && t < nv * 4) {
            a += dpp_f64<0xB1>(a);
            a += dpp_f64<0x4E>(a);
        }
        lds_barrier();
    }
    return a;
}

template <int NT, int HT>
__device__ __forceinline__ double block_pass(double* s_mem, const double (&oI)[NT], const double (&oQ)[NT],
                                             int tid, unsigned sel)
{
    if constexpr (GNSS_RED) return block_tree<NT>(s_mem, oI, oQ, tid, sel);
    constexpr int T = kTrkThreads;
    double* red = s_mem;
    double* red2 = s_mem + 2 * HT * T;
#pragma unroll
    for (int s = 0; s < NT; s++) {
        if ((sel >> s) & 1u) {
            const int q = __builtin_popcount(sel & ((1u << s) - 1u));
            red[(2 * q) * T + tid] = oI[s];
            red[(2 * q + 1) * T + tid] = oQ[s];
        }
    }
    lds_barrier();
    const int nv = 2 * __builtin_popcount(sel);
    for (int e = tid; e < nv * 32; e += T) {
        const double* r = red + (e >> 5) * T + (e & 31) * 8;
        double x = r[0];
#pragma unroll
        for (int k = 1; k < 8; k++) x += r[k];
        red2[e] = x;
    }
    lds_barrier();
    double a = 0.0;
    if (tid < nv * 4) {
        const double* r = red2 + (tid >> 2) * 32 + (tid & 3) * 8;
        a = r[0];
#pragma unroll
        for (int k = 1; k < 8; k++) a += r[k];
        a += dpp_f64<0xB1>(a);
        a += dpp_f64<0x4E>(a);
    }
    lds_barrier();
    return a;
}

template <int NV> constexpr int chan_lanes()
{
    return 16 * NV <= kTrkThreads ? 16 : 8 * NV <= kTrkThreads ? 8 : 4;
}

template <int L, class Load>
__device__ __forceinline__ double channel_sum_l(int bpc, int tid, Load load)
{
    const int v = tid / L, q = tid % L;
    double a = 0.0;
#pragma unroll 4
    for (int k = q; k < bpc; k += L) a += load(k, v);
    a += dpp_f64<0xB1>(a);
    a += dpp_f64<0x4E>(a);
    if constexpr (L >= 8) a += dpp_f64<0x141>(a);
    if constexpr (L == 16) a += dpp_f64<0x140>(a);
    return a;
}

template <int NV, class Load>
__device__ __forceinline__ double channel_sum(int bpc, int tid, Load load)
{
    constexpr int L = chan_lanes<NV>();
    const int v = tid / L, q = tid % L;
    double a = 0.0;
#pragma unroll 4
    for (int k = q; k < bpc; k += L) a += load(k, v);
    a += dpp_f64<0xB1>(a);
    a += dpp_f64<0x4E>(a);
    if constexpr (L >= 8) a += dpp_f64<0x141>(a);
    if constexpr (L == 16) a += dpp_f64<0x140>(a);
    return a;
}

template <int NT, int SUB, bool DIVIDE, int FMT = 0>
__global__ __launch_bounds__(kTrkThreads) void track_step_kernel(const TrkParams* __restrict__ pp,
                                                                const TrkBuffers* __restrict__ bp, int bpc)
{
    const TrkParams& p = *pp;
    const TrkBuffers& b = *bp;
    constexpr int M = 8 * SUB;
    constexpr int NV = 2 * NT;
    constexpr int T = kTrkThreads;
    static_assert(M <= kLaneMax, "lane span exceeds the rotation table");
    const int ch = blockIdx.x / bpc;
    const int blk = blockIdx.x - ch * bpc;
    const int tid = threadIdx.x, lane = tid & 63, wv = tid >> 6;

    constexpr int kSlot = 8 * T * 2;
    constexpr int kRed = red_words<red_taps<NT>()>();
    __shared__ __attribute__((aligned(16))) double s_mem[kSlot > kRed ? kSlot : kRed];
    __shared__ double s_fin[NV];
    __shared__ int s_last;
    __shared__ TrkChan s_c;
    __shared__ double2 s_zero;

    g_desc* dp = (g_desc*)(b.desc + ch);
    g_chan* cp = (g_chan*)(b.chan + ch);
    unsigned long long* srow = kProbe && b.stamps && ch == 0 ? stamp_row(b) : nullptr;
    if (srow && tid == 0) stamp_max(srow, 8 + blk, wall_clock64());
    const int64_t g_first = dp->g_first, g_last = dp->g_last;
    const int64_t g0 = g_first + ((int64_t)blk * T + tid) * SUB;
    const int8_t* iq = b.iq - p.buf_base;
    const int bad = dp->bad ? dp->bad : dp->bad_tap;
    constexpr int GB = FMT == 1 ? 2 : 1;
    int4 raw[SUB * GB];
#pragma unroll
    for (int j = 0; j < SUB; j++) {
        const int64_t gj = g0 + j <= g_last ? g0 + j : g_last;
#pragma unroll
        for (int h = 0; h < GB; h++)
            raw[GB * j + h] = bad ? make_int4(0, 0, 0, 0) : ld_g16(iq + 16 * GB * gj + 16 * h);
    }
    const unsigned cabits = lane < 32 ? ((g_cu32*)b.ca_bits)[ch * 32 + lane] : 0u;
    constexpr int kChanWords = (int)(sizeof(TrkChan) / 8);
    if (tid < kChanWords)
        reinterpret_cast<uint64_t*>(&s_c)[tid] = ((const g_u64*)cp)[tid];

    if (cp->status != GNSS_OK) return;
    if (!dp->phaseC && dp->Index + 1 > cp->n1_target) return;
    if (bad || dp->d * M >= 1.0) {
        if (blk == 0 && tid == 0) b.chan[ch].status = bad ? bad : GNSS_EINDEX;
        return;
    }
    double oI[NT], oQ[NT];
    if (kProbe && (p.probe & 2)) {
#pragma unroll
        for (int s = 0; s < NT; s++) { oI[s] = (double)raw[0].x; oQ[s] = 0.0; }
    } else {
        if (tid == 0) s_zero = make_double2(0.0, 0.0);
        __syncthreads();
        lane_correlate<NT, SUB, DIVIDE, false, FMT>(p, dp, RegRaw<SUB * GB>{raw}, 8 * g0 - dp->A, cabits,
                                        reinterpret_cast<double2*>(s_mem) + tid, &s_zero, oI, oQ);
    }

    __syncthreads();
    const double bsum = block_partial<NT>(s_mem, oI, oQ, tid);
    if (srow && tid == 0) stamp_max(srow, 8 + kMaxBpc + blk, wall_clock64());
    double* allp = b.partial + (int64_t)ch * bpc * NV;
    if (tid < NV * 4 && (tid & 3) == 0) st_sc1(allp + (int64_t)blk * NV + (tid >> 2), bsum);
    if constexpr (NV * 4 > 64) {
        asm volatile("s_waitcnt vmcnt(0)" ::: "memory");
        lds_barrier();
    }
    if (wv == 0) {
        asm volatile("s_waitcnt vmcnt(0)" ::: "memory");
        if (lane == 0) {
            const int g = blockIdx.x & 7;
            const int first = ((g - (ch * bpc) % 8) % 8 + 8) % 8;
            const unsigned cnt = first < bpc ? (unsigned)((bpc - 1 - first) / 8 + 1) : 0u;
            unsigned* sub = b.arrive + (ch * kArrivePerChan + g) * kArriveStride;
            unsigned* top = b.arrive + (ch * kArrivePerChan + 8) * kArriveStride;
            if (srow) stamp_max(srow, 8 + 2 * kMaxBpc + blk, wall_clock64());
            int last = 0;
            if (bpc <= 32) {
                if (atomic_add_agent(top, 1u) ==
                    (unsigned)bpc - 1) {
                    store_agent(top, 0u);
                    last = 1;
                }
            } else if (atomic_add_agent(sub, 1u) ==
                       cnt - 1) {
                store_agent(sub, 0u);
                const unsigned ngroups = bpc < 8 ? (unsigned)bpc : 8u;
                if (atomic_add_agent(top, 1u) ==
                    ngroups - 1) {
                    store_agent(top, 0u);
                    last = 1;
                }
            }
            s_last = last;
        }
    }
    __syncthreads();
    if (!s_last) return;

    if (srow && tid == 0) stamp_max(srow, 3, wall_clock64());
    double csum = 0.0;
    constexpr int CL = chan_lanes<NV>();
    if (tid < CL * NV)
        csum = channel_sum<NV>(bpc, tid, [&](int k, int v) { return ld_sc1(allp + (int64_t)k * NV + v); });
    StepOut o;
    o.n = dp->n;
    o.delayValue = dp->delayValue;
    o.remSample = dp->remSample;
    o.remChip = dp->remChip_next;
    o.remPhase = dp->remPhase_next;
    o.pdi = dp->pdi;
    o.phaseC = dp->phaseC;
    const bool dbg = b.dbg_sums || (kProbe && (p.probe & 1));
    if (tid < CL * NV && tid % CL == 0) {
        const int v = tid / CL;
        if (dbg) {
            if (b.dbg_sums) b.dbg_sums[ch * NV + v] = csum;
        } else {
            s_fin[v] = o.phaseC ? -csum : csum;
        }
    }
    if (dbg) return;
    __syncthreads();
    if (srow && tid == 0) stamp_max(srow, 4, wall_clock64());
    const LoopUpd u = loop_update_i(p, s_c, s_fin[2 * p.iE], s_fin[2 * p.iE + 1], s_fin[2 * p.iP],
                                  s_fin[2 * p.iP + 1], s_fin[2 * p.iL], s_fin[2 * p.iL + 1], o.pdi,
                                  o.phaseC);
    NcoState nx;
    nx.remChip = o.remChip;
    nx.remPhase = o.remPhase;
    nx.codeFreq = u.codeFreq;
    nx.carrierFreq = u.carrierFreq;
    nx.numSample = o.n;
    nx.pos = s_c.pos + p.bps * o.n;
    nx.Index = s_c.Index + (o.phaseC ? 10 : 1);
    if (wv == 0 || wv == 3) {
        if (kProbe && (p.probe & 8)) return;
        if (srow && wv == 0 && lane == 0) stamp_max(srow, 5, wall_clock64());
// ... 128 lines not shown
                          int base2, unsigned tag2, unsigned* dst2, int pid, int np, unsigned* err)
{
    const int n = n1 + n2;
    unsigned long long todo = 0;
    if (pid >= 0)
        for (int k = 0, e = pid; e < n; k++, e += np) todo |= 1ull << k;
    unsigned long long t0 = 0;
    int late = 0;
    while (todo) {
        for (int k = 0; (todo >> k) != 0; k++) {
            if (!((todo >> k) & 1ull)) continue;
            const int e = pid + k * np;
            const bool first = e < n1;
            const int e2 = first ? e : e - n1;
            const u32x4 v = __builtin_amdgcn_raw_buffer_load_b128(r, ((first ? base1 : base2) + e2) * 16, 0, kPolSc1);
            const unsigned tg = first ? tag1 : tag2;
            if (v.y == tg && v.w == tg) {
                unsigned* d = first ? dst1 : dst2;
                d[2 * e2] = v.x;
                d[2 * e2 + 1] = v.z;
                todo &= ~(1ull << k);
            }
        }
        if (!todo) break;
        if (++late >= 64) {
            const unsigned long long t = wall_clock64();
            if (!t0) t0 = t;
            else if (t - t0 > 200000000ull) { atomicExch(err, 1u); break; }
            late = 0;
        }
    }
    __shared__ unsigned s_vote2[kTrkThreads / 64];
    const unsigned any_left = __ballot(todo != 0) != 0ull ? 1u : 0u;
    if ((threadIdx.x & 63) == 0) s_vote2[threadIdx.x >> 6] = any_left;
    lds_barrier();
    unsigned v = 0;
#pragma unroll
    for (int w = 0; w < kTrkThreads / 64; w++) v |= s_vote2[w];
    return v == 0;
}

__device__ bool census(unsigned* w, int tid)
{
    __shared__ int s_go;
    if (tid == 0) {
        unsigned* arrive = w + 1;
        unsigned* state = w + 2;
        if (atomic_add_agent(arrive, 1u) == gridDim.x - 1)
            atomicCAS(state, 0u, 1u);
        const unsigned long long t0 = wall_clock64();
        unsigned st;
        while ((st = __hip_atomic_load((g_u32*)state, __ATOMIC_RELAXED, __HIP_MEMORY_SCOPE_AGENT)) == 0) {
            if (wall_clock64() - t0 > 2000000ull) atomicCAS(state, 0u, 2u);
            __builtin_amdgcn_s_sleep(2);
        }
        if (st == 2) atomicCAS(w, 0u, 2u);
        s_go = st == 1;
    }
    __syncthreads();
    return s_go != 0;
}

template <int SUB>
__device__ __forceinline__ void prefetch_raw(const int8_t* iq, int64_t g0, int64_t gmax, int4* s_raw,
                                             int tid)
{
    const int wbase = tid & ~63;
#pragma unroll
    for (int j = 0; j < SUB; j++) {
        int64_t gj = g0 + j;
        gj = gj < gmax ? gj : gmax;
        __builtin_amdgcn_global_load_lds((__attribute__((address_space(1))) void*)(iq + 16 * gj),
                                         (__attribute__((address_space(3))) void*)(s_raw + j * kTrkThreads + wbase),
                                         16, 0, 0);
    }
}

#ifndef GNSS_DEFER
#define GNSS_DEFER 0
#endif
#ifndef GNSS_WPE_TAPS
#define GNSS_WPE_TAPS 2
#endif
template <int NT, int SUB, bool DIVIDE, bool VB = false>
__global__ __launch_bounds__(kTrkThreads) __attribute__((amdgpu_waves_per_eu(NT > 3 ? GNSS_WPE_TAPS : 3, NT > 3 ? GNSS_WPE_TAPS : 3))) void track_run_kernel(const TrkParams* __restrict__ pp,
                                                               const TrkBuffers* __restrict__ bp, int bpc,
                                                               int vpb, int nsteps, unsigned tag0)
{
    const TrkParams& p = *pp;
    const TailK tk = tail_k(p);
    const TrkBuffers& b = *bp;
    constexpr int M = 8 * SUB;
    constexpr int NV = 2 * NT;
    constexpr int T = kTrkThreads;
    static_assert(M <= kLaneMax, "lane span exceeds the rotation table");
    const int vpb_ = VB ? vpb : 1;
    const int pbpc = (bpc + vpb_ - 1) / vpb_;
    const bool xl = GNSS_XCD_LOCAL == 1 && !VB && p.nch == 8;
    const bool cul = GNSS_XCD_LOCAL == 2 && !VB && p.nch == 8 && pbpc == 96;
    const int ch = xl ? (int)(blockIdx.x & 7) : cul ? (int)((blockIdx.x & 255) >> 5) : (int)(blockIdx.x / pbpc);
    const int pblk = xl ? (int)(blockIdx.x >> 3)
                    : cul ? (int)((blockIdx.x & 31) * 3 + (blockIdx.x >> 8)) : (int)(blockIdx.x - ch * pbpc);
    const int blk = pblk * vpb_;
    const int nvb = VB ? (bpc - blk < vpb_ ? bpc - blk : vpb_) : 1;
    const int tid = threadIdx.x, lane = tid & 63, wv = tid >> 6;
    const bool io = pblk == 0;

    constexpr int kSlot = 8 * T * 2;
    constexpr int kRed = red_words<run_red_taps<NT>()>();
    constexpr int kPart = run_bpc_cap(NT) * NV;
    constexpr bool kDefer = GNSS_DEFER && NT > 3;
    constexpr bool kWave1 = GNSS_DEFER == 2 && kDefer && !VB;
    static_assert(!kWave1 || GNSS_RED == 0, "GNSS_DEFER 2 needs GNSS_RED 0");
    constexpr int kPwD = run_bpc_cap(NT) * 8 + 2 * NT;
    constexpr int kStage = 2 * (NT - 1) * T;
    constexpr int kMemW = kWave1 ? kPwD + kStage + 2 * NT * 32 : 0;
    constexpr int kMem1 = kSlot > kRed ? kSlot : kRed;
    constexpr int kMem0 = kMem1 > kMemW ? kMem1 : kMemW;
    constexpr int kMem = kMem0 > kPart + 16 * NV ? kMem0 : kPart + 16 * NV;
    __shared__ __attribute__((aligned(16))) double s_mem[kMem];
    __shared__ __attribute__((aligned(16))) int4 s_raw[SUB * T];
    __shared__ __attribute__((aligned(16))) StepDesc s_d[2];
    __shared__ __attribute__((aligned(16))) TrkChan s_c;
    __shared__ StepOut s_o;
    __shared__ LoopUpd s_u;
    __shared__ double s_fin[NV];
    __shared__ double s_taps[GNSS_MAX_TAPS], s_post[GNSS_MAX_TAPS];
    __shared__ double2 s_zero;

    if (!census(b.run_err, tid)) return;
    g_chan* cp = (g_chan*)(b.chan + ch);
    if (cp->status != GNSS_OK) return;
    const int64_t n1_target = cp->n1_target;
    const int8_t* iq = b.iq - p.buf_base;
    const int64_t gmax = (p.buf_base + p.buf_len) / 16 - 1;
    const unsigned cabits = ca_bits_ext(lane < 32 ? ((g_cu32*)b.ca_bits)[ch * 32 + lane] : 0u, lane);
    const __amdgpu_buffer_rsrc_t pg = __builtin_amdgcn_make_buffer_rsrc(
        b.pgran + (int64_t)ch * 2 * gran_per_chan(NT), (short)0, gran_per_chan(NT) * 16, kBufRsrcWord3);
    constexpr int kChanWords = (int)(sizeof(TrkChan) / 8);

    constexpr int CL = chan_lanes<NV>();
    constexpr int HT = run_red_taps<NT>();
    struct DeferCfg {
        unsigned selA, selB;
        int NA, nBv, hb, own_lo, own_n, bneg;
        int64_t bslot;
        int vmap[kDefer ? NV : 1];
    };
    __shared__ DeferCfg s_df;
    typedef __attribute__((address_space(3))) volatile const int lds_vint;
    typedef __attribute__((address_space(3))) volatile const long long lds_vi64;
    auto dfi = [&](const int& f) { return uni((int)*(lds_vint*)&f); };
    auto NA_ = [&]() { return kDefer ? dfi(s_df.NA) : NV; };
    auto own_n_ = [&]() { return kDefer ? dfi(s_df.own_n) : 0; };
    const bool dob = kDefer && b.taps_rec != nullptr;
    if constexpr (kDefer) {
        if (tid == 0) {
            unsigned selA = 0, selB = 0;
            for (int s = 0; s < NT; s++) {
                if (s == tk.iE || s == tk.iP || s == tk.iL) selA |= 1u << s;
                else selB |= 1u << s;
            }
            const int nA = __builtin_popcount(selA), nB = __builtin_popcount(selB);
            const int nBv = 2 * nB, npass = (nB + HT - 1) / HT;
            int own_lo = 0, own_n = 0;
            if (dob && nBv > 0) {
                const int c = (nBv + pbpc - 1) / pbpc;
                const int nown = (nBv + c - 1) / c;
                const int r = ((pblk - 4) % pbpc + pbpc) % pbpc;
                if (r < nown) {
                    own_lo = r * c;
                    own_n = nBv - own_lo < c ? nBv - own_lo : c;
                }
            }
            s_df.selA = selA;
            s_df.selB = selB;
            s_df.NA = 2 * nA;
            s_df.nBv = nBv;
            s_df.hb = npass > 0 ? (nB + npass - 1) / npass : 1;
            s_df.own_lo = own_lo;
            s_df.own_n = own_n;
            s_df.bneg = 0;
            s_df.bslot = 0;
            for (int s = 0; s < NT; s++) {
                const unsigned below = (1u << s) - 1u;
                const int v = ((selA >> s) & 1u) ? 2 * __builtin_popcount(selA & below)
                                                 : 2 * nA + 2 * __builtin_popcount(selB & below);
                s_df.vmap[v] = 2 * s;
                s_df.vmap[v + 1] = 2 * s + 1;
            }
        }
// ... 86 lines not shown
            a += dpp_f64<0x4E>(a);
            if ((lane & 3) == 0)
                publish16(pg, gran_region_b(NT) + (step & 3) * gran_slot_b(NT) + (lane >> 2) * bpc + blk, a,
                          tag0 + step + 1);
        }
    };
    auto flush = [&]() {
        if (wv == 1) {
            unsigned long long* fr = kProbe && (GNSS_FLUSH_PROBE & 2) && b.stamps && ch == 0 && io && lane == 0
                                         ? b.stamps + (size_t)(s_now % kStampSlots) * kStampRow : nullptr;
            if (fr) fr[2000] = wall_clock64();
            if (lane == 0 && !(GNSS_FLUSH_PROBE & 1)) {
                if (dio) {
                    if (!pre_ok) {
                        asm volatile("s_waitcnt vmcnt(0)" ::: "memory");
                        const g_i64* dvp = (const g_i64*)(b.dvpre + (int64_t)ch * (p.rec_cap + 1));
                        const int64_t cols = record_cols(p, s_c, s_o.phaseC);
                        pre[1] = cols < s_c.nstep + 1 ? dvp[cols] : 0;
                    }
                    pre[0] = dvrun;
                    write_record_i(p, b, ch, s_c, s_o, s_u, s_fin, pre, duty_b == duty_a ? 3 : 1);
                    dvrun += s_o.delayValue;
                }
                else if (pblk == duty_b) write_record_i(p, b, ch, s_c, s_o, s_u, s_fin, nullptr, 2);
            }
            if (fr) {
                fr[2001] = wall_clock64();
                write_record_i(p, b, ch, s_c, s_o, s_u, s_fin, pre, 3);
                fr[2002] = wall_clock64();
            }
            if (pblk == duty_b && b.taps_rec && lane < NA_() && s_c.slot < p.rec_cap) {
                const int v = kDefer ? s_df.vmap[lane] : lane;
                ((g_dbl*)b.taps_rec)[((int64_t)ch * p.rec_cap + s_c.slot) * NV + v] = s_fin[v];
            }
            if (kDefer && lane == 0) {
                s_df.bslot = s_c.slot;
                s_df.bneg = s_o.phaseC;
            }
            if (lane == 0) update_state_inplace(p, b, ch, s_c, s_o, s_u, s_fin, pblk == duty_c);
        }
        pend = false;
        pre_ok = false;
    };
    const unsigned long long t_start = kProbe ? wall_clock64() : 0ull;
    for (int s = 0; s < nsteps; s++) {
        s_now = s;
        const StepDesc& D = s_d[cur];
        const int bad = D.bad ? D.bad : D.bad_tap;
        const bool stop = !D.phaseC && D.Index + 1 > n1_target;
        if (bad || stop || D.d * M >= 1.0 || (GNSS_QCAP && NT > kQcapMax && D.d > tk.qcap_dmax)) {
            const bool had = pend;
            if (pend) flush();
            if (had) defer_final(s - 1);
            if (io && tid == 64) desc_rem(tk, &s_d[cur]);
            __syncthreads();
            if (io) {
                if (tid == 0 && !stop) s_c.status = bad ? bad : GNSS_EINDEX;
                __syncthreads();
                if (tid < kChanWords)
                    reinterpret_cast<uint64_t*>(b.chan + ch)[tid] = reinterpret_cast<const uint64_t*>(&s_c)[tid];
                for (int e = tid; e < kDescWords; e += T)
                    reinterpret_cast<unsigned*>(b.desc + ch)[e] = reinterpret_cast<const unsigned*>(&D)[e];
            }
            return;
        }
        const int64_t A = uni(D.A), n = uni(D.n);
        unsigned long long* srow = kProbe && b.stamps && ch == 0 && (io || pblk == pbpc - 1)
                                       ? b.stamps + (size_t)(s % kStampSlots) * kStampRow + (io ? 0 : 5) : nullptr;
        if (srow && tid == 0) srow[0] = wall_clock64();
        unsigned long long* brow = kProbe && b.stamps && ch == 0 ? b.stamps + (size_t)(s % kStampSlots) * kStampRow : nullptr;
        if (brow && tid == 0) brow[40 + blk] = wall_clock64();

        for (int jv = 0; jv < nvb; jv++) {
            const int vb = blk + jv;
            switch ((kProbe && (p.probe & 64)) ? ch % 3 : (kProbe && (p.probe & 128)) ? 0 : (s + ch) % 3) {
            case 0: __builtin_amdgcn_s_setprio(0); break;
            case 1: __builtin_amdgcn_s_setprio(1); break;
            default: __builtin_amdgcn_s_setprio(2); break;
            }
            {
                const int64_t g0 = uni(D.g_first) + ((int64_t)vb * T + tid) * SUB;
                asm volatile("s_waitcnt vmcnt(0)" ::: "memory");
                double oI[NT], oQ[NT];
                lane_correlate<NT, SUB, DIVIDE, true, 0>(p, &D, LdsRaw{s_raw + tid}, 8 * g0 - A, cabits,
                                                      reinterpret_cast<double2*>(s_mem) + tid, &s_zero, oI, oQ,
                                                      s_post);
                __syncthreads();
                if (pend && dio && wv == 1 && lane == 0 && jv == 0) {
                    asm volatile("s_waitcnt vmcnt(0)" ::: "memory");
                    const g_i64* dvp = (const g_i64*)(b.dvpre + (int64_t)ch * (p.rec_cap + 1));
                    const int64_t cols = record_cols(p, s_c, s_o.phaseC);
                    pre[1] = cols < s_c.nstep + 1 ? dvp[cols] : 0;
                    pre_ok = true;
                }
                if (VB && jv + 1 < nvb)
                    prefetch_raw<SUB>(iq, uni(D.g_first) + ((int64_t)(vb + 1) * T + tid) * SUB, gmax, s_raw, tid);
                __builtin_amdgcn_s_setprio(3);
                if (srow && tid == 0) srow[1] = wall_clock64();
                if (brow && tid == 0) brow[40 + 256 + vb] = wall_clock64();
                if constexpr (!kDefer) {
                    const double bsum = block_partial<NT, HT>(s_mem, oI, oQ, tid);
                    if (tid < NV * 4 && (tid & 3) == 0)
                        publish16(pg, ((s & 1) * kMaxBpcRun + vb) * NV + (tid >> 2), bsum, tag0 + s + 1);
                } else {
                    const double ba = block_pass<NT, HT>(s_mem, oI, oQ, tid, (unsigned)dfi(*(const int*)&s_df.selA));
                    const int NA = NA_();
                    if (tid < NA * 4 && (tid & 3) == 0)
                        publish16(pg, ((s & 1) * kMaxBpcRun + vb) * NA + (tid >> 2), ba, tag0 + s + 1);
                    if (kWave1 && dob) {
                        double* stg = s_mem + kPwD;
                        const unsigned sb = (unsigned)dfi(*(const int*)&s_df.selB);
#pragma unroll
                        for (int s2 = 0; s2 < NT; s2++)
                            if ((sb >> s2) & 1u) {
                                const int r = __builtin_popcount(sb & ((1u << s2) - 1u));
                                stg[(2 * r) * T + tid] = oI[s2];
                                stg[(2 * r + 1) * T + tid] = oQ[s2];
                            }
                        lds_barrier();
                    } else if (dob) {
                        const int hb = dfi(s_df.hb), nB = dfi(s_df.nBv) / 2;
                        for (int ps = 1; (ps - 1) * hb < nB; ps++) {
                            const unsigned sel = sel_pass(ps);
                            const double bb = block_pass<NT, HT>(s_mem, oI, oQ, tid, sel);
                            if (tid < 2 * __builtin_popcount(sel) * 4 && (tid & 3) == 0)
                                publish16(pg, gran_region_b(NT) + (s & 3) * gran_slot_b(NT) +
                                                  (2 * (ps - 1) * hb + (tid >> 2)) * bpc + vb,
                                          bb, tag0 + s + 1);
                        }
                    }
                }
                if (srow && tid == 0) srow[2] = wall_clock64();
                if (kProbe && b.stamps && ch == 0 && tid == 0) {
                    unsigned long long* r = b.stamps + (size_t)(s % kStampSlots) * kStampRow;
                    atomicMax(r + 23, wall_clock64());
                    atomicMax(r + 24, ~wall_clock64());
                }
            }
        }

        if (wv == (io ? GNSS_IO_DR_WAVE : 2) && lane == 0) desc_rem(tk, &s_d[cur]);
        const bool bsw = kDefer && pend && own_n_() > 0;
        if (pend) {
            if (srow && tid == 64) srow[16] = wall_clock64();
            if (brow && tid == 64) brow[40 + 1024 + blk] = wall_clock64();
            flush();
            if (srow && tid == 64) srow[17] = wall_clock64();
            if (brow && tid == 64) brow[40 + 1280 + blk] = wall_clock64();
        }

        unsigned* pw = reinterpret_cast<unsigned*>(s_mem);
        {
            int pid = GNSS_SWEEP_IO_ALL || !dsw ? tid : (wv == 1 ? -1 : tid - (wv > 1 ? 64 : 0));
            int np = GNSS_SWEEP_IO_ALL || !dsw ? 4 * 64 : 3 * 64;
            if (kWave1 && dob) {
                const int bw = dsw ? 3 : 1;
                if (wv == bw) defer_reduce(s);
                const int rank = wv == 0 ? 0 : wv - 1;
                pid = (wv == bw || wv == 1) ? -1 : rank * 64 + lane;
                np = dsw ? 2 * 64 : 3 * 64;
            }
            if constexpr (!kDefer) {
                if (!sweep16<(NT > 3 ? GNSS_SWEEP_BATCH : 1)>(pg, bpc * NV, tag0 + s + 1, pw, pid, np, b.run_err,
                                                               (s & 1) * kMaxBpcRun * NV))
                    return;
            } else {
                const int NA = NA_();
// ... 127 lines not shown
    const TrkBuffers& b = *bp;
    const int ch = blockIdx.x;
    __shared__ int s_first;
    if (threadIdx.x == 0) s_first = 0x7fffffff;
    __syncthreads();
    TrkChan& c = b.chan[ch];
    if (c.status != GNSS_OK) return;
    const double* P = b.p_i_1ms + (int64_t)ch * b.n1;
    const int64_t len = b.n1;
    auto sgn = [](double x) { return (x > 0) - (x < 0); };
    int mine = 0x7fffffff;
    for (int64_t i = 7 + (int64_t)threadIdx.x; i <= len - 1; i += (int64_t)blockDim.x) {
        const int si = sgn(P[i - 1]);
        int before = 1;
        for (int j = 6; j >= 1; j--) before &= sgn(P[i - j - 1]) != si ? 1 : 0;
        int stop = 0;
        if (before) {
            int k = 1;
            for (; k <= 17; k++) {
                if (i + k > len) { stop = 1; break; }
                if (sgn(P[i + k - 1]) != si) break;
            }
            if (k > 17 && i >= 600) stop = 1;
        }
        if (stop && (int)i < mine) mine = (int)i;
    }
    if (mine != 0x7fffffff) atomicMin(&s_first, mine);
    __syncthreads();
    if (threadIdx.x != 0) return;
    const int64_t i = s_first;
    int cx = 0;
    if (i != 0x7fffffff) {
        const int si = sgn(P[i - 1]);
        bool ok = true;
        for (int j = 6; j >= 1 && ok; j--) ok = sgn(P[i - j - 1]) != si;
        for (int j = 1; j <= 17 && ok; j++) {
            if (i + j > len) { c.status = GNSS_EINDEX; return; }
            ok = sgn(P[i + j - 1]) == si;
        }
        cx = (int)(i % 20) - 1;
    }
    c.countinx = cx;
    c.n1_target = b.n1 + cx;
}

__global__ void track_phase_c_init_kernel(const TrkParams* __restrict__ pp, const TrkBuffers* __restrict__ bp,
                                          int64_t skip)
{
    const TrkParams& p = *pp;
    const TrkBuffers& b = *bp;
    const int ch = blockIdx.x;
    __shared__ TrkChan s_c;
    if (threadIdx.x == 0) {
        TrkChan c = b.chan[ch];
        if (c.status == GNSS_OK) {
            const int cx = c.countinx;
            if (cx < 0) {
                c = b.snap[ch];
                c.countinx = cx;
                c.n1_target = b.n1 + cx;
            }
            const int64_t S = (int64_t)p.S;
            c.pos = (int64_t)((S - c.codedelay0 + 1 + (skip + b.n1 + cx) * S) *
                              (int64_t)p.dataBytesPerSample);
            c.index_int = 0;
            c.snrIndex = 1;
            c.nstep = 0;
            c.Index = b.n1 + cx;
            c.slot = b.n1 + cx;
            b.dvpre[(int64_t)ch * (p.rec_cap + 1)] = 0;
            b.chan[ch] = c;
        }
        s_c = c;
    }
    __syncthreads();
    const TrkChan c = s_c;
    if (c.status == GNSS_OK) prepare_desc_block(p, nco_of(c), 10, 1, b.desc + ch);
}

hipError_t launch_track_step(const TrkParams& p, const TrkBuffers& b, const TrkDev& d, int bpc, int sub,
                             hipStream_t s)
{
    dim3 grid(p.nch * bpc), block(kTrkThreads);
#define GNSS_STEP(NT_, SUB_, DIV_, FMT_)                                                       \
    if (p.ntaps == NT_ && sub == SUB_ && (p.exact_div != 0) == DIV_ && p.fmt == FMT_) {        \
        hipLaunchKernelGGL((track_step_kernel<NT_, SUB_, DIV_, FMT_>), grid, block, 0, s, d.p, d.b, bpc); \
        return hipGetLastError();                                                              \
    }
    GNSS_STEP(3, 1, false, 0) GNSS_STEP(3, 2, false, 0) GNSS_STEP(3, 3, false, 0) GNSS_STEP(3, 4, false, 0)
    GNSS_STEP(11, 1, false, 0) GNSS_STEP(11, 2, false, 0) GNSS_STEP(11, 3, false, 0) GNSS_STEP(11, 4, false, 0)
    GNSS_STEP(3, 1, true, 0) GNSS_STEP(11, 1, true, 0)
    GNSS_STEP(25, 1, false, 0) GNSS_STEP(25, 3, false, 0) GNSS_STEP(25, 1, true, 0)
    GNSS_STEP(3, 1, false, 1) GNSS_STEP(3, 3, false, 1) GNSS_STEP(11, 1, false, 1) GNSS_STEP(11, 3, false, 1)
    GNSS_STEP(3, 1, true, 1) GNSS_STEP(11, 1, true, 1)
#undef GNSS_STEP
    return hipErrorInvalidValue;
}

hipError_t launch_track_run(const TrkParams& p, const TrkBuffers& b, const TrkDev& d, int bpc, int vpb, int sub,
                            int nsteps, unsigned tag0, hipStream_t s)
{
    if (vpb < 1 || bpc < 1) return hipErrorInvalidValue;
    dim3 grid(p.nch * ((bpc + vpb - 1) / vpb)), block(kTrkThreads);
#define GNSS_RUN(NT_, SUB_, DIV_)                                                              \
    if (p.ntaps == NT_ && sub == SUB_ && (p.exact_div != 0) == DIV_ && vpb == 1) {            \
        hipLaunchKernelGGL((track_run_kernel<NT_, SUB_, DIV_, false>), grid, block, 0, s, d.p, d.b, bpc, vpb, \
                           nsteps, tag0);                                                      \
        return hipGetLastError();                                                              \
    }
#define GNSS_RUNV(NT_, SUB_, DIV_)                                                             \
    if (p.ntaps == NT_ && sub == SUB_ && (p.exact_div != 0) == DIV_ && vpb > 1) {             \
        hipLaunchKernelGGL((track_run_kernel<NT_, SUB_, DIV_, true>), grid, block, 0, s, d.p, d.b, bpc, vpb, \
                           nsteps, tag0);                                                      \
        return hipGetLastError();                                                              \
    }
    GNSS_RUN(3, 1, false) GNSS_RUN(3, 2, false) GNSS_RUN(3, 3, false) GNSS_RUN(3, 4, false)
    GNSS_RUN(11, 1, false) GNSS_RUN(11, 2, false) GNSS_RUN(11, 3, false) GNSS_RUN(11, 4, false)
    GNSS_RUN(3, 1, true) GNSS_RUN(11, 1, true)
    GNSS_RUNV(3, 1, false) GNSS_RUNV(3, 3, false) GNSS_RUNV(11, 1, false) GNSS_RUNV(11, 3, false)
#undef GNSS_RUN
#undef GNSS_RUNV
    return hipErrorInvalidValue;
}

int track_run_blocks_per_cu(const TrkParams& p, int sub, bool vb)
{
    int nb = 0;
#define GNSS_OCC(NT_, SUB_, DIV_, VB_)                                                         \
    if (p.ntaps == NT_ && sub == SUB_ && (p.exact_div != 0) == DIV_ && vb == VB_) {            \
        if (hipOccupancyMaxActiveBlocksPerMultiprocessor(                                      \
                &nb, reinterpret_cast<const void*>(track_run_kernel<NT_, SUB_, DIV_, VB_>),     \
                kTrkThreads, 0) != hipSuccess)                                                 \
            nb = 0;                                                                            \
        return nb;                                                                             \
    }
    GNSS_OCC(3, 1, false, false) GNSS_OCC(3, 2, false, false) GNSS_OCC(3, 3, false, false)
    GNSS_OCC(3, 4, false, false) GNSS_OCC(11, 1, false, false) GNSS_OCC(11, 2, false, false)
    GNSS_OCC(11, 3, false, false) GNSS_OCC(11, 4, false, false) GNSS_OCC(3, 1, true, false)
    GNSS_OCC(11, 1, true, false)
    GNSS_OCC(3, 1, false, true) GNSS_OCC(3, 3, false, true) GNSS_OCC(11, 1, false, true)
    GNSS_OCC(11, 3, false, true)
#undef GNSS_OCC
    return 0;
}

__global__ void track_expand_kernel(const double* __restrict__ src, int64_t rec_cap, int stride, int nf,
                                    const int64_t* __restrict__ job, double* __restrict__ dst, int64_t ML,
                                    int64_t n10, int ntaps)
{
    const int i = blockIdx.y / nf, f = blockIdx.y - i * nf;
    const int64_t n1 = job[2 * i], c = job[2 * i + 1];
    const double* s = src + (int64_t)i * rec_cap * stride + f;
    const int fo = ntaps ? (f & 1) * ntaps + (f >> 1) : f;
    double* o = dst + (c * nf + fo) * ML;
    for (int64_t k = (int64_t)blockIdx.x * blockDim.x + threadIdx.x; k < ML; k += (int64_t)gridDim.x * blockDim.x) {
        double v = 0.0;
        if (k < n1) v = s[k * stride];
        else if (k < n1 + 10 * n10) v = s[(n1 + (k - n1) / 10) * stride];
        o[k] = v;
    }
}

hipError_t launch_track_expand(const double* src, int64_t rec_cap, int stride, int nf, int nch,
                               const int64_t* job, double* dst, int64_t ML, int64_t n10, int ntaps,
                               hipStream_t s)
{
    const int64_t chunks = (ML + 255) / 256;
    hipLaunchKernelGGL(track_expand_kernel, dim3((unsigned)(chunks < 64 ? chunks : 64), (unsigned)(nch * nf)),
                       dim3(256), 0, s, src, rec_cap, stride, nf, job, dst, ML, n10, ntaps);
    return hipGetLastError();
}

hipError_t launch_track_prepare(const TrkParams& p, const TrkBuffers& b, const TrkDev& d, int pdi,
                                int phaseC, hipStream_t s)
{
    hipLaunchKernelGGL(track_prepare_kernel, dim3(p.nch), dim3(192), 0, s, d.p, d.b, pdi, phaseC);
    return hipGetLastError();
}

hipError_t launch_track_snapshot(const TrkParams& p, const TrkBuffers& b, const TrkDev& d, hipStream_t s)
{
    hipLaunchKernelGGL(track_snapshot_kernel, dim3((p.nch + 63) / 64), dim3(64), 0, s, d.b, p.nch);
    return hipGetLastError();
}

hipError_t launch_track_bitedge(const TrkParams& p, const TrkBuffers& b, const TrkDev& d, hipStream_t s)
{
    hipLaunchKernelGGL(track_bitedge_kernel, dim3(p.nch), dim3(256), 0, s, d.b, p.nch);
    return hipGetLastError();
}

hipError_t launch_track_phase_c_init(const TrkParams& p, const TrkBuffers& b, const TrkDev& d,
                                     int64_t skip, hipStream_t s)
{
    hipLaunchKernelGGL(track_phase_c_init_kernel, dim3(p.nch), dim3(192), 0, s, d.p, d.b, skip);
    return hipGetLastError();
}

}
```

assignment-for-aae6102_gnss-sdr_amd/sdr.py:

```python
from __future__ import annotations

import ctypes as C
import math
from types import SimpleNamespace

import numpy as np

from . import abi


def initParameters(fileRoute: str | None = None):
    file = SimpleNamespace(fileName="Opensky", fileRoute=fileRoute, skip=5000, skiptimeVT=100,
                           dataType=2, dataPrecision=1, data=None, dev=None)
    signal = SimpleNamespace(IF=4.58e6, Fs=58e6, Fc=1575.42e6, codeFreqBasis=1.023e6, ms=1e-3)
    signal.Sample = math.ceil(signal.Fs * signal.ms)
    signal.codelength = signal.codeFreqBasis * signal.ms
    acq = SimpleNamespace(prnList=list(range(1, 33)), freqStep=500, freqMin=-10000, datalen=20, L=10)
    acq.freqNum = int(2 * abs(acq.freqMin) / acq.freqStep + 1)
    track = SimpleNamespace(CorrelatorSpacing=0.5, DLLBW=2, DLLDamp=0.707, DLLGain=0.1, PLLBW=15,
                            PLLDamp=0.707, PLLGain=0.25, msToProcessCT_1ms=1000,
                            msToProcessCT_10ms=40000, ctPOS=3000, msToProcessVT=5000, pdi=1)
    solu = SimpleNamespace(iniPos=[22.328444770087565 / 180 * math.pi,
                                   114.1713630049711 / 180 * math.pi, 4],
                           navSolPeriod=20, mode=2)
    cmn = SimpleNamespace(doy=171, vtEnable=1, mltCorrON=[1, 0], cSpeed=299792458, equip="stereo")
    return file, signal, acq, track, solu, cmn


class Context:

    def __init__(self, device: int = 0, devices=None):
        self.lib = abi.load()
        h = C.c_void_p()
        if devices is not None:
            devs = [int(d) for d in devices]
            arr = (C.c_int * len(devs))(*devs)
            st = self.lib.gnss_ctx_create_multi(arr, len(devs), C.byref(h))
            if st != abi.OK:
                raise abi.GnssError(st, f"gnss_ctx_create_multi(devices={devs}) failed")
            device = devs[0]
        else:
            st = self.lib.gnss_ctx_create(int(device), C.byref(h))
            if st != abi.OK:
                raise abi.GnssError(st, f"gnss_ctx_create(device={device}) failed")
        self.h = h
        self.device = device
        self.devices = list(devices) if devices is not None else [device]

    @property
    def members(self) -> int:
        return int(self.lib.gnss_ctx_members(self.h))

    def close(self):
        if getattr(self, "h", None):
            self.lib.gnss_ctx_destroy(self.h)
            self.h = None

    def __del__(self):
        try:
            self.close()
        except Exception:
            pass

    def check(self, st):
        if st != abi.OK:
            raise abi.GnssError(st, (self.lib.gnss_last_error(self.h) or b"").decode())
        return st

    def timing(self) -> dict:
        t = abi.GnssTiming()
        self.check(self.lib.gnss_last_timing(self.h, C.byref(t)))
        return {f: getattr(t, f) for f, _ in abi.GnssTiming._fields_}

    def set_profiling(self, on: bool):
        self.check(self.lib.gnss_ctx_set_profiling(self.h, 1 if on else 0))

    def set_window(self, nbytes: int):
        self.check(self.lib.gnss_ctx_set_window(self.h, int(nbytes)))

    def set_option(self, key: int, value: int):
        self.check(self.lib.gnss_ctx_set_option(self.h, int(key), int(value)))

    def drop_record(self, dev=None):
        if dev is None:
            ptr = None
        else:
            v = getattr(dev, "ptr", dev)
            ptr = v.value if isinstance(v, C.c_void_p) else int(v)
        self.check(self.lib.gnss_ctx_drop_record(self.h, C.c_void_p(ptr)))

    @property
    def resident_records(self) -> int:
        return int(self.lib.gnss_ctx_resident_records(self.h))

    def set_acq_precision(self, fp64: bool):
        self.check(self.lib.gnss_ctx_set_acq_precision(self.h, 1 if fp64 else 0))


class DeviceRecord:

    def __init__(self, ctx: Context, nbytes: int):
        self.ctx = ctx
        self.nbytes = int(nbytes)
        p = C.c_void_p()
        ctx.check(ctx.lib.gnss_dev_alloc(ctx.h, C.c_uint64(self.nbytes), C.byref(p)))
        self.ptr = p

    @classmethod
    def from_host(cls, ctx: Context, data: np.ndarray):
        data = np.ascontiguousarray(data, dtype=np.int8)
        r = cls(ctx, data.nbytes)
        ctx.check(ctx.lib.gnss_dev_upload(ctx.h, r.ptr, data.ctypes.data_as(C.c_void_p),
                                          C.c_uint64(data.nbytes)))
        return r

    def upload(self, data: np.ndarray, offset: int = 0):
        data = np.ascontiguousarray(data, dtype=np.int8)
        dst = C.c_void_p(self.ptr.value + int(offset))
        self.ctx.check(self.ctx.lib.gnss_dev_upload(self.ctx.h, dst, data.ctypes.data_as(C.c_void_p),
                                                    C.c_uint64(data.nbytes)))

    def download(self, offset: int = 0, nbytes: int | None = None) -> np.ndarray:
        n = self.nbytes - offset if nbytes is None else int(nbytes)
        out = np.empty(n, dtype=np.int8)
        src = C.c_void_p(self.ptr.value + int(offset))
        self.ctx.check(self.ctx.lib.gnss_dev_download(self.ctx.h, out.ctypes.data_as(C.c_void_p),
                                                      src, C.c_uint64(n)))
        return out

    def free(self):
        if self.ptr:
            self.ctx.lib.gnss_dev_free(self.ctx.h, self.ptr)
            self.ptr = None


_default_ctx: Context | None = None


def default_context() -> Context:
    global _default_ctx
    if _default_ctx is None:
        _default_ctx = Context(0)
    return _default_ctx


def to_c_file(file):
    f = abi.GnssFile()
    keep = []
    path = getattr(file, "fileRoute", None)
    data = getattr(file, "data", None)
    dev = getattr(file, "dev", None)
    if dev is not None:
        f.dev_data = dev.ptr
        f.nbytes = dev.nbytes
    elif data is not None:
        arr = np.ascontiguousarray(data) if isinstance(data, np.ndarray) else np.asarray(data, np.int8)
        arr = arr.reshape(-1).view(np.int8)
        keep.append(arr)
        f.data = arr.ctypes.data
        f.nbytes = arr.nbytes
    elif path:
        f.path = str(path).encode()
    else:
        raise abi.GnssError(abi.EARG, "file has no fileRoute, data or dev record")
# ... 625 lines not shown
```

include/gnss_mi355x.h:

```cpp
#ifndef GNSS_MI355X_H
#define GNSS_MI355X_H

#include <stdint.h>
#include <stddef.h>

#ifdef __cplusplus
extern "C" {
#endif

#define GNSS_ABI_VERSION 13

#define GNSS_OK         0
#define GNSS_ENODATA    1
#define GNSS_EIO        2
#define GNSS_EARG       3
#define GNSS_EDEVICE    4
#define GNSS_EINDEX     5

#define GNSS_MAX_SV     64
#define GNSS_MAX_TAPS   32


typedef struct gnss_file {
    const char   *path;
// ... 50 lines not shown
    int32_t msToProcessCT_1ms;
    int32_t msToProcessCT_10ms;
    int32_t        n_taps;
    const double  *tap_offsets;
    int32_t        n_chan;
    const int32_t *chan;
} gnss_track;

enum gnss_track_field {
    GNSS_F_P_i = 0, GNSS_F_P_q, GNSS_F_E_i, GNSS_F_E_q, GNSS_F_L_i, GNSS_F_L_q,
    GNSS_F_PLLdiscri, GNSS_F_DLLdiscri, GNSS_F_codedelay, GNSS_F_remChip,
    GNSS_F_codeFreq, GNSS_F_carrierFreq, GNSS_F_remPhase, GNSS_F_remSample,
    GNSS_F_numSample, GNSS_F_delayValue, GNSS_F_absoluteSample, GNSS_F_codedelay2,
    GNSS_NFIELDS
};

#define GNSS_F_carrError               GNSS_F_PLLdiscri
#define GNSS_F_codeError               GNSS_F_DLLdiscri
#define GNSS_F_carrFreq                GNSS_F_carrierFreq
#define GNSS_F_remCarrPhase            GNSS_F_remPhase
#define GNSS_F_absoluteSampleCodedelay GNSS_F_remSample

#define GNSS_OUT_DEVICE 1
typedef struct gnss_track_out {
    int64_t  max_len;
    double  *rec;
    double  *taps;
    int64_t *len;
    int32_t *countinx;
    double  *CN0_Eph;
    int32_t  cn0_cap;
    int32_t  cn0_rows;
    int32_t  flags;
    int32_t  reserved;
} gnss_track_out;

typedef struct gnss_timing {
    double acq_ms;
    double acq_corr_ms;
    double acq_fine_ms;
    double track_ms;
    double track_kernel_ms;
    int64_t track_launches;
    int64_t track_channel_samples;
    int64_t acq_hypothesis_samples;
    double h2d_ms;
    double  track10_kernel_ms;
    int64_t track10_launches;
    int64_t track10_channel_samples;
    int64_t h2d_bytes;
    int64_t track_segments;
} gnss_timing;

typedef struct gnss_ctx gnss_ctx;

int         gnss_abi_version(void);
const char *gnss_strerror(int status);

int  gnss_ctx_create(int device, gnss_ctx **out);
#define GNSS_MAX_DEVICES 16
int  gnss_ctx_create_multi(const int *devices, int n, gnss_ctx **out);
int  gnss_ctx_drop_record(gnss_ctx *ctx, const void *dev_ptr);
int  gnss_ctx_resident_records(const gnss_ctx *ctx);
int  gnss_device_count(void);
int  gnss_ctx_members(const gnss_ctx *ctx);
void gnss_ctx_destroy(gnss_ctx *ctx);
const char *gnss_last_error(const gnss_ctx *ctx);
int  gnss_last_timing(const gnss_ctx *ctx, gnss_timing *out);
int  gnss_ctx_set_profiling(gnss_ctx *ctx, int enable);
int  gnss_ctx_set_acq_precision(gnss_ctx *ctx, int fp64);
int  gnss_ctx_set_window(gnss_ctx *ctx, uint64_t bytes);
#define GNSS_OPT_FORCE_SUB    0
#define GNSS_OPT_NO_PERSIST   1
#define GNSS_OPT_FORCE_VPB    2
#define GNSS_OPT_ACQ_ROCFFT   3
#define GNSS_OPT_FINE_ROCFFT  4
#define GNSS_OPT_ACQ_BATCH    5
#define GNSS_OPT_ACQ_FUSED    6
#define GNSS_OPT_ACQ_RING     7
#define GNSS_OPT_ACQ_PIPE     8
#define GNSS_OPT_VT_BLOCKS    9
#define GNSS_OPT_FORCE_PEER   10
#define GNSS_OPT_VT_SPAN      11
#define GNSS_OPT_COUNT        12
int  gnss_ctx_set_option(gnss_ctx *ctx, int key, int64_t value);

int  gnss_dev_alloc(gnss_ctx *ctx, uint64_t nbytes, void **dev_ptr);
int  gnss_dev_free(gnss_ctx *ctx, void *dev_ptr);
int  gnss_dev_upload(gnss_ctx *ctx, void *dev_dst, const void *host_src, uint64_t nbytes);
int  gnss_dev_download(gnss_ctx *ctx, void *host_dst, const void *dev_src, uint64_t nbytes);

int gnss_acquisition(gnss_ctx *ctx, const gnss_file *file, const gnss_signal *signal,
                     const gnss_acq *acq, gnss_acquired *out, gnss_acq_diag *diag);

int gnss_tracking_ct(gnss_ctx *ctx, const gnss_file *file, const gnss_signal *signal,
                     const gnss_track *track, const gnss_acquired *acquired,
                     gnss_track_out *out);

int gnss_tracking_ct_pos(gnss_ctx *ctx, const gnss_file *file, const gnss_signal *signal,
                         const gnss_track *track, const gnss_acquired *acquired, int32_t ctPOS,
                         const int32_t *countinx, gnss_track_out *out);

#define GNSS_MC_TAPS 25

int gnss_tracking_ct_multicorr(gnss_ctx *ctx, const gnss_file *file, const gnss_signal *signal,
                               const gnss_track *track, const gnss_acquired *acquired,
                               int32_t datalength, gnss_track_out *out);
int gnss_tracking_ct_mc(gnss_ctx *ctx, const gnss_file *file, const gnss_signal *signal,
                        const gnss_track *track, const gnss_acquired *acquired, int32_t msPosCT,
                        int32_t pdi, gnss_track_out *out);

enum gnss_eph_field {
    GNSS_E_TOW = 0, GNSS_E_TOW1, GNSS_E_sfb, GNSS_E_sfb1, GNSS_E_weeknum, GNSS_E_N, GNSS_E_health,
    GNSS_E_IODC, GNSS_E_TGD, GNSS_E_toc, GNSS_E_af2, GNSS_E_af1, GNSS_E_af0, GNSS_E_IODE2, GNSS_E_Crs,
    GNSS_E_deltan, GNSS_E_M0, GNSS_E_Cuc, GNSS_E_ecc, GNSS_E_Cus, GNSS_E_sqrta, GNSS_E_toe, GNSS_E_Cic,
    GNSS_E_omegae, GNSS_E_Cis, GNSS_E_i0, GNSS_E_Crc, GNSS_E_w, GNSS_E_omegadot, GNSS_E_IODE3,
    GNSS_E_idot, GNSS_E_updatetime, GNSS_E_updatetime_tow,
    GNSS_EPH_NFIELDS
};

typedef struct gnss_nav_out {
    int32_t  eph_cap;
    double  *eph;
    int32_t *eph_len;
    int32_t *updateflag;
    int64_t *nav1;
    int64_t *sfb1;
} gnss_nav_out;

int gnss_navi_decode(const gnss_acquired *acquired, const double *P_i, const int64_t *len,
                     int64_t stride, gnss_nav_out *out);

int gnss_correlate_step(gnss_ctx *ctx, const gnss_file *file, const gnss_signal *signal,
                        int prn, int pdi, double remChip, double codeFreq, double carrierFreq,
                        double remPhase, int64_t pos_bytes, int n_taps, const double *taps,
                        double *sums_out, int64_t *numSample_out);

typedef struct gnss_vt_chan {
    int32_t prn;
    int32_t pad;
    int64_t file_ptr;
    double  remChip;
    double  remCarrPhase;
    double  codeFreq;
    double  carrFreq;
    double  carrFreqBasis;
    double  oldCarrNco, oldCarrError;
    int32_t index_int;
    int32_t snrIndex;
    double  Zk[20];
} gnss_vt_chan;

typedef struct gnss_vt_out {
    double  E_i, E_q, P_i, P_q, L_i, L_q;
    double  carrError, codeError, carrNco;
    double  remChip, remCarrPhase, codeFreq, carrFreq;
    int64_t numSample, absoluteSample;
    double  codedelay;
    double  CN0;
    int32_t cn0_row;
    int32_t status;
    double  deltaPr;
    double  prRate;
    double  sv_vel[3];
} gnss_vt_out;

int gnss_tracking_vt_run(gnss_ctx *ctx, const gnss_file *file, const gnss_signal *signal,
                         const gnss_track *track, int32_t pdi, int32_t n, int32_t nsteps,
// ... 166 lines not shown
```

Baseline: 390,500.

## Add register-capture lane correlator path for three-tap tracking, dropping LDS slot buffer

Adds a register-capture variant of the tracking lane correlator for tap sets with at most three taps. Partial sums at tap boundaries are captured into registers with masked inline asm instead of going through a per-thread LDS slot buffer, and a fallback loop handles lanes that have more than one capture point. A host-side boundary count picks this path at runtime, and an option lets it be forced on or off. The intent is to remove LDS traffic and LDS footprint, at the cost of extra register pressure and a rarely taken recompute loop.

```diff
diff --git a/assignment-for-aae6102_gnss-sdr_amd/abi.py b/assignment-for-aae6102_gnss-sdr_amd/abi.py
--- a/assignment-for-aae6102_gnss-sdr_amd/abi.py
+++ b/assignment-for-aae6102_gnss-sdr_amd/abi.py
@@ -249,6 +249,8 @@
                                       C.POINTER(C.c_double), C.POINTER(GnssVtMcOut)]),
     "gnss_vt_mc_nav_update": (C.c_int, [C.POINTER(GnssVtNav), C.POINTER(C.c_double), C.POINTER(C.c_double),
                                         C.POINTER(C.c_double), C.POINTER(GnssVtNavSol)]),
+    "gnss_lane_boundaries": (C.c_int, [C.POINTER(C.c_double), C.POINTER(C.c_double), C.c_int, C.c_int, C.c_double]),
+    "gnss_ctx_lane_path": (C.c_int, [C.c_void_p]),
 }
 
 LIB_PATH = os.path.join(os.path.dirname(os.path.abspath(__file__)), "lib", "libgnss_mi355x.so")
@@ -257,7 +259,7 @@
 LOADED_PATH = None
 
 (OPT_FORCE_SUB, OPT_NO_PERSIST, OPT_FORCE_VPB, OPT_ACQ_ROCFFT, OPT_FINE_ROCFFT, OPT_ACQ_BATCH, OPT_ACQ_FUSED,
- OPT_ACQ_RING, OPT_ACQ_PIPE, OPT_VT_BLOCKS, OPT_FORCE_PEER, OPT_VT_SPAN) = range(12)
+ OPT_ACQ_RING, OPT_ACQ_PIPE, OPT_VT_BLOCKS, OPT_FORCE_PEER, OPT_VT_SPAN, OPT_SLOT_PATH) = range(13)
 MAX_DEVICES = 16
 
 
diff --git a/assignment-for-aae6102_gnss-sdr_amd/csrc/gnss_api.cpp b/assignment-for-aae6102_gnss-sdr_amd/csrc/gnss_api.cpp
--- a/assignment-for-aae6102_gnss-sdr_amd/csrc/gnss_api.cpp
+++ b/assignment-for-aae6102_gnss-sdr_amd/csrc/gnss_api.cpp
@@ -44,6 +44,7 @@
     int acq_fp64 = 1;
     uint64_t window = 0;
     int64_t opt[GNSS_OPT_COUNT] = {};
+    int lane_path = 0;
     std::vector<gnss_ctx*> members;
     bool member = false;
     int fail_chan = -1;
@@ -907,6 +908,8 @@
     if (!ctx || key < 0 || key >= GNSS_OPT_COUNT) return GNSS_EARG;
     if (key == GNSS_OPT_VT_BLOCKS && (value < 0 || value > GNSS_VT_MAX_BLOCKS))
         return fail(ctx, GNSS_EARG, "GNSS_OPT_VT_BLOCKS outside 0..%d", GNSS_VT_MAX_BLOCKS);
+    if (key == GNSS_OPT_SLOT_PATH && (value < 0 || value > 2))
+        return fail(ctx, GNSS_EARG, "GNSS_OPT_SLOT_PATH outside 0..2");
     if (key == GNSS_OPT_VT_SPAN && (value < 0 || value > kVtSpan))
         return fail(ctx, GNSS_EARG, "GNSS_OPT_VT_SPAN outside 0..%d", kVtSpan);
     ctx->opt[key] = value;
@@ -1402,6 +1405,7 @@
     int cus = 0;
     HIP_TRY(hipDeviceGetAttribute(&cus, hipDeviceAttributeMultiprocessorCount, ctx->device));
     P.qcap_dmax = cps_max;
+    P.regcap = regcap_mask(P, cps_max, ctx->opt[GNSS_OPT_SLOT_PATH]);
     auto qcap_ok = [&](int sub) {
         return !GNSS_QCAP || P.ntaps <= 3 ||
                max_taps_in_lane(P.taps, P.tap_post, P.ntaps, 8 * sub, cps_max) <= kQcapMax;
@@ -1425,6 +1429,7 @@
     bool persist1 = vpb1 > 0, persist10 = vpb10 > 0;
     if (const char* pr = probe_env("GNSS_PROBE")) P.probe = atoi(pr);
     const int bpc1 = bpc_for(1, sub1), bpc10 = bpc_for(10, sub10);
+    ctx->lane_path = lane_regcap(P, sub1) && lane_regcap(P, sub10);
     if (bpc10 > kMaxBpc) return fail(ctx, GNSS_EARG, "Sample too large for the step geometry");
 
     std::vector<TrkChan> ch0((size_t)nch);
@@ -1844,6 +1849,14 @@
     return tracking_impl(ctx, file, sg, tr, acq, out, &pc);
 }
 
+int gnss_lane_boundaries(const double* taps, const double* post, int n_taps, int lane_samples, double cps_max)
+{
+    if (!taps || n_taps < 1 || n_taps > GNSS_MAX_TAPS || lane_samples < 1 || !(cps_max > 0.0)) return -1;
+    return lane_boundaries(taps, post, n_taps, lane_samples, cps_max);
+}
+
+int gnss_ctx_lane_path(const gnss_ctx* ctx) { return ctx ? ctx->lane_path : 0; }
+
 int gnss_correlate_step(gnss_ctx* ctx, const gnss_file* file, const gnss_signal* sg, int prn, int pdi,
                         double remChip, double codeFreq, double carrierFreq, double remPhase,
                         int64_t pos_bytes, int n_taps, const double* taps, double* sums_out,
@@ -1893,6 +1906,8 @@
     if (const int v = (int)ctx->opt[GNSS_OPT_FORCE_SUB]) {
         if (v >= 2 && v <= 4 && !P.exact_div && 8.0 * v * codeFreq / sg->Fs < 1.0) sub = v;
     }
+    P.regcap = regcap_mask(P, codeFreq / sg->Fs, ctx->opt[GNSS_OPT_SLOT_PATH]);
+    ctx->lane_path = lane_regcap(P, sub);
     const int bpc = (int)std::ceil(((S * pdi * 1.01 + 64) / 8.0 + 2) / ((double)kTrkThreads * sub));
     DevBuf d_chan, d_desc, d_ca, d_part, d_arrive, d_sums;
     HIP_TRY(d_chan.alloc(sizeof(TrkChan)));
diff --git a/assignment-for-aae6102_gnss-sdr_amd/csrc/gnss_internal.h b/assignment-for-aae6102_gnss-sdr_amd/csrc/gnss_internal.h
--- a/assignment-for-aae6102_gnss-sdr_amd/csrc/gnss_internal.h
+++ b/assignment-for-aae6102_gnss-sdr_amd/csrc/gnss_internal.h
@@ -231,6 +231,7 @@
     int32_t chip_off;
     int32_t given;
     double tap_post[GNSS_MAX_TAPS];
+    int32_t regcap;
 };
 
 constexpr int kLaneMax = 32;
@@ -330,6 +331,47 @@
         best = c > best ? c : best;
     }
     return best;
+}
+inline int lane_boundaries(const double* taps, const double* post, int n, int M, double dmax)
+{
+    const double w = (M - 1) * dmax + 1e-9;
+    auto off = [&](int s) { return taps[s] + (post ? post[s] : 0.0); };
+    auto same = [&](int a, int b) {
+        const double f = off(a) - off(b), r = f - floor(f);
+        return r < 1e-9 || r > 1.0 - 1e-9;
+    };
+    int best = 0;
+    for (int a = 0; a < n; a++) {
+        int c = 0, multi = 0;
+        for (int b = 0; b < n; b++) {
+            bool first = true;
+            int size = 0;
+            for (int e = 0; e < n; e++) {
+                if (!same(b, e)) continue;
+                if (e < b) first = false;
+                size++;
+            }
+            if (!first) continue;
+            double f = off(b) - off(a);
+            f -= floor(f);
+            if (f < w || f > 1.0 - 1e-9) {
+                c++;
+                multi += size > 1;
+            }
+        }
+        c += multi > 1 ? multi : 1;
+        best = c > best ? c : best;
+    }
+    return best;
+}
+constexpr int kRegCapMax = 2;
+inline bool lane_regcap(const TrkParams& p, int sub) { return p.ntaps <= 3 && ((p.regcap >> sub) & 1) != 0; }
+inline int regcap_mask(const TrkParams& p, double dmax, int64_t force)
+{
+    int m = 0;
+    for (int sub = 1; sub <= 4 && force != 1 && p.ntaps <= 3; sub++)
+        if (force == 2 || lane_boundaries(p.taps, p.tap_post, p.ntaps, 8 * sub, dmax) <= kRegCapMax) m |= 1 << sub;
+    return m;
 }
 constexpr int kDeferSlots = 4;
 constexpr int gran_region_b(int ntaps) { return ntaps > 3 ? 2 * kMaxBpcRun * 6 : 0; }
diff --git a/assignment-for-aae6102_gnss-sdr_amd/csrc/track.hip b/assignment-for-aae6102_gnss-sdr_amd/csrc/track.hip
--- a/assignment-for-aae6102_gnss-sdr_amd/csrc/track.hip
+++ b/assignment-for-aae6102_gnss-sdr_amd/csrc/track.hip
@@ -1,4 +1,8 @@
 #include "gnss_internal.h"
+
+#include <cstddef>
+#include <type_traits>
+#include <utility>
 
 namespace gnss {
 
@@ -619,6 +623,21 @@
     const int4* p;
     __device__ __forceinline__ int4 get(int j) const { return p[j * kTrkThreads]; }
 };
+typedef __attribute__((address_space(3))) const char lds_cchar;
+typedef __attribute__((address_space(3))) const double lds_cdbl;
+typedef double dbl2v __attribute__((ext_vector_type(2)));
+typedef __attribute__((address_space(3))) const dbl2v lds_cdbl2;
+
+template <class F, int... I>
+__device__ __forceinline__ void static_for_seq(F&& f, std::integer_sequence<int, I...>)
+{
+    (f(std::integral_constant<int, I>{}), ...);
+}
+template <int N, class F>
+__device__ __forceinline__ void static_for(F&& f)
+{
+    static_for_seq(f, std::make_integer_sequence<int, N>{});
+}
 
 #ifndef GNSS_CORR_PROBE
 #define GNSS_CORR_PROBE 0
@@ -645,16 +664,29 @@
 #ifndef GNSS_SWP
 #define GNSS_SWP 0
 #endif
-#ifndef GNSS_REGCAP
-#define GNSS_REGCAP 0
-#endif
 #ifndef GNSS_PHI_REG
 #define GNSS_PHI_REG 0
 #endif
 #ifndef GNSS_TAPWIN
 #define GNSS_TAPWIN 1
 #endif
-template <int NT, int SUB, bool DIVIDE, bool RELOAD, int FMT, class Desc, class Raw>
+template <int MS>
+__device__ __forceinline__ void capture_at(int capA, double& run_r, double& run_i, double& pre_r,
+                                           double& pre_i, double& kbt, unsigned& adr)
+{
+    unsigned long long sv;
+    asm volatile("s_mov_b64 %[sv], exec\n\t"
+                 "v_cmpx_eq_u32_e32 vcc, %[m], %[cap]\n\t"
+                 "v_mov_b64 %[pr], %[rr]\n\t"
+                 "v_mov_b64 %[pi], %[ri]\n\t"
+                 "s_mov_b64 exec, %[sv]"
+                 : [pr] "+v"(pre_r), [pi] "+v"(pre_i), [rr] "+v"(run_r), [ri] "+v"(run_i), [sv] "=&s"(sv),
+                   "+v"(kbt), "+v"(adr)
+                 : [cap] "v"(capA), [m] "n"(MS)
+                 : "vcc");
+}
+
+template <int NT, int SUB, bool DIVIDE, bool RELOAD, int FMT, bool REGC = false, class Desc, class Raw>
 __device__ __forceinline__ void lane_correlate(const TrkParams& p, const Desc* dp, const Raw& raw,
                                                int64_t ks, unsigned cabits, double2* myslot,
                                                const double2* zero, double (&oI)[NT], double (&oQ)[NT],
@@ -662,7 +694,9 @@
 {
     constexpr int M = 8 * SUB;
     constexpr int T = kTrkThreads;
-    constexpr bool QC = RELOAD && (GNSS_QCAP == 2 || (GNSS_QCAP && NT > 3));
+    constexpr bool QC = RELOAD && GNSS_QCAP && NT > 3;
+    static_assert(!REGC || (NT <= 3 && !QC && GNSS_CORR_PROBE == 0 && !GNSS_SWP && !GNSS_PHI_REG),
+                  "register capture: the <= 3-tap product forms");
     if constexpr ((GNSS_CORR_PROBE & 8) != 0) {
 #pragma unroll
         for (int s = 0; s < NT; s++) { oI[s] = 0.0; oQ[s] = 0.0; }
@@ -804,7 +838,6 @@
         mu_i = uni(dp->mu_i);
     }
 
-    constexpr bool RC = GNSS_REGCAP && !QC && NT <= 3;
     double dhi_l = 0.0, dlo_l = 0.0;
     if constexpr (GNSS_PHI_REG) {
         dhi_l = uni(dp->dhi);
@@ -812,6 +845,155 @@
     }
     double Wpipe = 0.0;
     if constexpr (GNSS_SWP) Wpipe = wave_at<DIVIDE>(kb + 1.0, f, phi0, Fs, rFs);
+    if constexpr (REGC) {
+        constexpr unsigned kPhi = (unsigned)offsetof(StepDesc, phi), kRcs = (unsigned)offsetof(StepDesc, rcs);
+        int capA = -1;
+#pragma unroll
+        for (int s = NT - 1; s >= 0; s--) capA = (cap[s] >= 0 && cap[s] < M - 1) ? cap[s] : capA;
+        double preA_r = 0.0, preA_i = 0.0;
+        double kbt = kb;
+        unsigned adr = 0u;
+        if constexpr (RELOAD) adr = (unsigned)(size_t)(lds_cchar*)dp;
+        auto table = [&](const int m, const unsigned ta, double& phm, double2& rcs) __attribute__((always_inline)) {
+            if constexpr (RELOAD) {
+                phm = *(lds_cdbl*)(size_t)(ta + kPhi + 8u * (unsigned)m);
+                const dbl2v v = *(lds_cdbl2*)(size_t)(ta + kRcs + 16u * (unsigned)m);
+                rcs = make_double2(v.x, v.y);
+            } else {
+                phm = dp->phi[m];
+                rcs = ld_rcs(dp, m);
+            }
+        };
+        auto rotation = [&](const int m, const double kbase, const double phm, const double2 rcs, double& rc,
+                            double& rs) __attribute__((always_inline)) {
+            const double W = wave_at<DIVIDE>(kbase + (double)m, f, phi0, Fs, rFs);
+            const double eta = (W - Wb) - phm;
+            rc = __builtin_fma(-eta, rcs.y, rcs.x);
+            rs = __builtin_fma(eta, rcs.x, rcs.y);
+        };
+        auto accumulate = [&](const double rc, const double rs, const double xr, const double xi, double& rr,
+                              double& ri) __attribute__((always_inline)) {
+            rr = __builtin_fma(xr, rc, rr);
+            rr = __builtin_fma(-xi, rs, rr);
+            ri = __builtin_fma(xr, rs, ri);
+            ri = __builtin_fma(xi, rc, ri);
+        };
+        double ph_n = 0.0, rc_n = 1.0, rs_n = 0.0;
+        double2 rcs_n = make_double2(1.0, 0.0);
+        table(1, adr, ph_n, rcs_n);
+        rotation(1, kbt, ph_n, rcs_n, rc_n, rs_n);
+        table(2, adr, ph_n, rcs_n);
+        static_for<SUB>([&](auto jc) __attribute__((always_inline)) {
+            constexpr int j = decltype(jc)::value;
+            constexpr int NW = FMT == 1 ? 8 : 4;
+            unsigned wd[NW];
+            const bool part = lo > 8 * j || hi < 8 * j + 8;
+            if constexpr (FMT == 1) {
+                const int4 ra = raw.get(2 * j), rb = raw.get(2 * j + 1);
+                wd[0] = (unsigned)ra.x; wd[1] = (unsigned)ra.y; wd[2] = (unsigned)ra.z; wd[3] = (unsigned)ra.w;
+                wd[4] = (unsigned)rb.x; wd[5] = (unsigned)rb.y; wd[6] = (unsigned)rb.z; wd[7] = (unsigned)rb.w;
+            } else {
+                const int4 rj = raw.get(j);
+                wd[0] = (unsigned)rj.x; wd[1] = (unsigned)rj.y; wd[2] = (unsigned)rj.z; wd[3] = (unsigned)rj.w;
+                if (part) {
+#pragma unroll
+                    for (int q = 0; q < 4; q++) {
+                        const int m0 = 8 * j + 2 * q;
+                        const unsigned k0 = (m0 >= lo && m0 < hi) ? 0x0000FFFFu : 0u;
+                        const unsigned k1 = (m0 + 1 >= lo && m0 + 1 < hi) ? 0xFFFF0000u : 0u;
+                        wd[q] &= k0 | k1;
+                    }
+                }
+            }
+            static_for<8>([&](auto mc) __attribute__((always_inline)) {
+                constexpr int mm = decltype(mc)::value, m = 8 * j + mm;
+                double xr, xi;
+                if constexpr (FMT == 1) {
+                    const unsigned word = wd[mm];
+                    xr = (double)(short)(word & 0xFFFFu) - mu_r;
+                    xi = (double)(short)(word >> 16) - mu_i;
+                    if (part && !(m >= lo && m < hi)) { xr = 0.0; xi = 0.0; }
+                } else {
+                    const unsigned word = wd[mm >> 1];
+                    constexpr int sh = (mm & 1) * 16;
+                    xr = (double)(int8_t)((word >> sh) & 0xFF);
+                    xi = (double)(int8_t)((word >> (sh + 8)) & 0xFF);
+                }
+                const double rc = rc_n, rs = rs_n;
+                if constexpr (m > 0 && m + 1 < M) {
+                    rotation(m + 1, kbt, ph_n, rcs_n, rc_n, rs_n);
+                    if constexpr (m + 2 < M) table(m + 2, adr, ph_n, rcs_n);
+                }
+                if constexpr (m > 0) {
+                    accumulate(rc, rs, xr, xi, run_r, run_i);
+                } else {
+                    run_r += xr;
+                    run_i += xi;
+                }
+                if constexpr (m < M - 1) capture_at<m>(capA, run_r, run_i, preA_r, preA_i, kbt, adr);
+            });
+        });
+        bool more = false;
+#pragma unroll
+        for (int s = 0; s < NT; s++) {
+            const int cs = cap[s];
+            more = more || (cs >= 0 && cs < M - 1 && cs != capA);
+            pre_r[s] = (cs < 0 ? 0.0 : cs == M - 1 ? run_r : preA_r) + 0.0;
+            pre_i[s] = (cs < 0 ? 0.0 : cs == M - 1 ? run_i : preA_i) + 0.0;
+        }
+        if (__builtin_amdgcn_ballot_w64(more) != 0ull) {
+            double r2 = 0.0, i2 = 0.0;
+            double q_r[NT], q_i[NT];
+#pragma unroll
+            for (int s = 0; s < NT; s++) { q_r[s] = 0.0; q_i[s] = 0.0; }
+#pragma unroll
+            for (int j = 0; j < SUB; j++)
+#pragma unroll 1
+            for (int mm = 0; mm < (j == SUB - 1 ? 7 : 8); mm++) {
+                const int m = 8 * j + mm;
+                double xr, xi;
+                if constexpr (FMT == 1) {
+                    const int4 ga = raw.get(2 * j), gb = raw.get(2 * j + 1);
+                    const int c = mm & 3;
+                    const int wa = c == 0 ? ga.x : c == 1 ? ga.y : c == 2 ? ga.z : ga.w;
+                    const int wb = c == 0 ? gb.x : c == 1 ? gb.y : c == 2 ? gb.z : gb.w;
+                    const unsigned word = (unsigned)(mm < 4 ? wa : wb);
+                    xr = (double)(short)(word & 0xFFFFu) - mu_r;
+                    xi = (double)(short)(word >> 16) - mu_i;
+                } else {
+                    const int4 g = raw.get(j);
+                    const int c = mm >> 1, sh = (mm & 1) * 16;
+                    const unsigned word = (unsigned)(c == 0 ? g.x : c == 1 ? g.y : c == 2 ? g.z : g.w);
+                    xr = (double)(int8_t)((word >> sh) & 0xFF);
+                    xi = (double)(int8_t)((word >> (sh + 8)) & 0xFF);
+                }
+                if (!(m >= lo && m < hi)) { xr = 0.0; xi = 0.0; }
+                if (m > 0) {
+                    double ph;
+                    double2 rcs;
+                    table(m, adr, ph, rcs);
+                    double rc, rs;
+                    rotation(m, kb, ph, rcs, rc, rs);
+                    accumulate(rc, rs, xr, xi, r2, i2);
+                } else {
+                    r2 += xr;
+                    i2 += xi;
+                }
+#pragma unroll
+                for (int s = 0; s < NT; s++) {
+                    const bool at = cap[s] == m;
+                    q_r[s] = at ? r2 : q_r[s];
+                    q_i[s] = at ? i2 : q_i[s];
+                }
+            }
+#pragma unroll
+            for (int s = 0; s < NT; s++) {
+                const bool in = cap[s] >= 0 && cap[s] < M - 1;
+                pre_r[s] = in ? q_r[s] + 0.0 : pre_r[s];
+                pre_i[s] = in ? q_i[s] + 0.0 : pre_i[s];
+            }
+        }
+    }
     auto subgroup = [&](const int j) {
         constexpr int NW = FMT == 1 ? 8 : 4;
         unsigned wd[NW];
@@ -881,19 +1063,12 @@
             if constexpr (QC) {
                 if ((cmask >> m) & 1u)
                     myslot[__builtin_popcount(cmask & ((1u << m) - 1u)) * T] = make_double2(run_r, run_i);
-            } else if constexpr (RC) {
-#pragma unroll
-                for (int s = 0; s < NT; s++) {
-                    const bool at = cap[s] == m;
-                    pre_r[s] = at ? run_r : pre_r[s];
-                    pre_i[s] = at ? run_i : pre_i[s];
-                }
             } else {
                 myslot[mm * T] = make_double2(run_r, run_i);
             }
             if constexpr (GNSS_SWP == 2) __builtin_amdgcn_sched_barrier(0);
         }
-        if constexpr (!QC && !RC) {
+        if constexpr (!QC) {
 #pragma unroll
             for (int s = 0; s < NT; s++) {
                 const unsigned idx = (unsigned)(cap[s] - 8 * j);
@@ -906,7 +1081,8 @@
 #ifndef GNSS_UNROLL_TAPS
 #define GNSS_UNROLL_TAPS 0
 #endif
-    if constexpr (RELOAD && ((NT > 3 && !GNSS_UNROLL_TAPS) || (RC && GNSS_REGCAP == 2))) {
+    if constexpr (REGC) {
+    } else if constexpr (RELOAD && NT > 3 && !GNSS_UNROLL_TAPS) {
 #pragma unroll 1
         for (int j = 0; j < SUB; j++) subgroup(j);
     } else if constexpr (RELOAD) {
@@ -1146,7 +1322,7 @@
     return a;
 }
 
-template <int NT, int SUB, bool DIVIDE, int FMT = 0>
+template <int NT, int SUB, bool DIVIDE, int FMT = 0, bool REGC = false>
 __global__ __launch_bounds__(kTrkThreads) void track_step_kernel(const TrkParams* __restrict__ pp,
                                                                 const TrkBuffers* __restrict__ bp, int bpc)
 {
@@ -1160,7 +1336,7 @@
     const int blk = blockIdx.x - ch * bpc;
     const int tid = threadIdx.x, lane = tid & 63, wv = tid >> 6;
 
-    constexpr int kSlot = 8 * T * 2;
+    constexpr int kSlot = REGC ? 0 : 8 * T * 2;
     constexpr int kRed = red_words<red_taps<NT>()>();
     __shared__ __attribute__((aligned(16))) double s_mem[kSlot > kRed ? kSlot : kRed];
     __shared__ double s_fin[NV];
@@ -1203,7 +1379,7 @@
     } else {
         if (tid == 0) s_zero = make_double2(0.0, 0.0);
         __syncthreads();
-        lane_correlate<NT, SUB, DIVIDE, false, FMT>(p, dp, RegRaw<SUB * GB>{raw}, 8 * g0 - dp->A, cabits,
+        lane_correlate<NT, SUB, DIVIDE, false, FMT, REGC>(p, dp, RegRaw<SUB * GB>{raw}, 8 * g0 - dp->A, cabits,
                                         reinterpret_cast<double2*>(s_mem) + tid, &s_zero, oI, oQ);
     }
 
@@ -1498,7 +1674,7 @@
 #ifndef GNSS_WPE_TAPS
 #define GNSS_WPE_TAPS 2
 #endif
-template <int NT, int SUB, bool DIVIDE, bool VB = false>
+template <int NT, int SUB, bool DIVIDE, bool VB = false, bool REGC = false>
 __global__ __launch_bounds__(kTrkThreads) __attribute__((amdgpu_waves_per_eu(NT > 3 ? GNSS_WPE_TAPS : 3, NT > 3 ? GNSS_WPE_TAPS : 3))) void track_run_kernel(const TrkParams* __restrict__ pp,
                                                                const TrkBuffers* __restrict__ bp, int bpc,
                                                                int vpb, int nsteps, unsigned tag0)
@@ -1522,7 +1698,7 @@
     const int tid = threadIdx.x, lane = tid & 63, wv = tid >> 6;
     const bool io = pblk == 0;
 
-    constexpr int kSlot = 8 * T * 2;
+    constexpr int kSlot = REGC ? 0 : 8 * T * 2;
     constexpr int kRed = red_words<run_red_taps<NT>()>();
     constexpr int kPart = run_bpc_cap(NT) * NV;
     constexpr bool kDefer = GNSS_DEFER && NT > 3;
@@ -1775,7 +1951,7 @@
                 const int64_t g0 = uni(D.g_first) + ((int64_t)vb * T + tid) * SUB;
                 asm volatile("s_waitcnt vmcnt(0)" ::: "memory");
                 double oI[NT], oQ[NT];
-                lane_correlate<NT, SUB, DIVIDE, true, 0>(p, &D, LdsRaw{s_raw + tid}, 8 * g0 - A, cabits,
+                lane_correlate<NT, SUB, DIVIDE, true, 0, REGC>(p, &D, LdsRaw{s_raw + tid}, 8 * g0 - A, cabits,
                                                       reinterpret_cast<double2*>(s_mem) + tid, &s_zero, oI, oQ,
                                                       s_post);
                 __syncthreads();
@@ -2069,9 +2245,14 @@
                              hipStream_t s)
 {
     dim3 grid(p.nch * bpc), block(kTrkThreads);
+    const bool regc = lane_regcap(p, sub);
 #define GNSS_STEP(NT_, SUB_, DIV_, FMT_)                                                       \
     if (p.ntaps == NT_ && sub == SUB_ && (p.exact_div != 0) == DIV_ && p.fmt == FMT_) {        \
-        hipLaunchKernelGGL((track_step_kernel<NT_, SUB_, DIV_, FMT_>), grid, block, 0, s, d.p, d.b, bpc); \
+        if (NT_ <= 3 && regc)                                                                  \
+            hipLaunchKernelGGL((track_step_kernel<NT_, SUB_, DIV_, FMT_, NT_ <= 3>), grid, block, 0, s, d.p, d.b, \
+                               bpc);                                                           \
+        else                                                                                   \
+            hipLaunchKernelGGL((track_step_kernel<NT_, SUB_, DIV_, FMT_>), grid, block, 0, s, d.p, d.b, bpc); \
         return hipGetLastError();                                                              \
     }
     GNSS_STEP(3, 1, false, 0) GNSS_STEP(3, 2, false, 0) GNSS_STEP(3, 3, false, 0) GNSS_STEP(3, 4, false, 0)
@@ -2089,16 +2270,25 @@
 {
     if (vpb < 1 || bpc < 1) return hipErrorInvalidValue;
     dim3 grid(p.nch * ((bpc + vpb - 1) / vpb)), block(kTrkThreads);
+    const bool regc = lane_regcap(p, sub);
 #define GNSS_RUN(NT_, SUB_, DIV_)                                                              \
     if (p.ntaps == NT_ && sub == SUB_ && (p.exact_div != 0) == DIV_ && vpb == 1) {            \
-        hipLaunchKernelGGL((track_run_kernel<NT_, SUB_, DIV_, false>), grid, block, 0, s, d.p, d.b, bpc, vpb, \
-                           nsteps, tag0);                                                      \
+        if (NT_ <= 3 && regc)                                                                  \
+            hipLaunchKernelGGL((track_run_kernel<NT_, SUB_, DIV_, false, NT_ <= 3>), grid, block, 0, s, d.p, d.b, \
+                               bpc, vpb, nsteps, tag0);                                        \
+        else                                                                                   \
+            hipLaunchKernelGGL((track_run_kernel<NT_, SUB_, DIV_, false>), grid, block, 0, s, d.p, d.b, bpc, \
+                               vpb, nsteps, tag0);                                             \
         return hipGetLastError();                                                              \
     }
 #define GNSS_RUNV(NT_, SUB_, DIV_)                                                             \
     if (p.ntaps == NT_ && sub == SUB_ && (p.exact_div != 0) == DIV_ && vpb > 1) {             \
-        hipLaunchKernelGGL((track_run_kernel<NT_, SUB_, DIV_, true>), grid, block, 0, s, d.p, d.b, bpc, vpb, \
-                           nsteps, tag0);                                                      \
+        if (NT_ <= 3 && regc)                                                                  \
+            hipLaunchKernelGGL((track_run_kernel<NT_, SUB_, DIV_, true, NT_ <= 3>), grid, block, 0, s, d.p, d.b, \
+                               bpc, vpb, nsteps, tag0);                                        \
+        else                                                                                   \
+            hipLaunchKernelGGL((track_run_kernel<NT_, SUB_, DIV_, true>), grid, block, 0, s, d.p, d.b, bpc, \
+                               vpb, nsteps, tag0);                                             \
         return hipGetLastError();                                                              \
     }
     GNSS_RUN(3, 1, false) GNSS_RUN(3, 2, false) GNSS_RUN(3, 3, false) GNSS_RUN(3, 4, false)
@@ -2113,11 +2303,13 @@
 int track_run_blocks_per_cu(const TrkParams& p, int sub, bool vb)
 {
     int nb = 0;
+    const bool regc = lane_regcap(p, sub);
 #define GNSS_OCC(NT_, SUB_, DIV_, VB_)                                                         \
     if (p.ntaps == NT_ && sub == SUB_ && (p.exact_div != 0) == DIV_ && vb == VB_) {            \
-        if (hipOccupancyMaxActiveBlocksPerMultiprocessor(                                      \
-                &nb, reinterpret_cast<const void*>(track_run_kernel<NT_, SUB_, DIV_, VB_>),     \
-                kTrkThreads, 0) != hipSuccess)                                                 \
+        const void* fn = NT_ <= 3 && regc                                                      \
+                             ? reinterpret_cast<const void*>(track_run_kernel<NT_, SUB_, DIV_, VB_, NT_ <= 3>) \
+                             : reinterpret_cast<const void*>(track_run_kernel<NT_, SUB_, DIV_, VB_>); \
+        if (hipOccupancyMaxActiveBlocksPerMultiprocessor(&nb, fn, kTrkThreads, 0) != hipSuccess) \
             nb = 0;                                                                            \
         return nb;                                                                             \
     }
diff --git a/assignment-for-aae6102_gnss-sdr_amd/sdr.py b/assignment-for-aae6102_gnss-sdr_amd/sdr.py
--- a/assignment-for-aae6102_gnss-sdr_amd/sdr.py
+++ b/assignment-for-aae6102_gnss-sdr_amd/sdr.py
@@ -80,6 +80,9 @@
 
     def set_option(self, key: int, value: int):
         self.check(self.lib.gnss_ctx_set_option(self.h, int(key), int(value)))
+
+    def lane_path(self) -> int:
+        return int(self.lib.gnss_ctx_lane_path(self.h))
 
     def drop_record(self, dev=None):
         if dev is None:
diff --git a/include/gnss_mi355x.h b/include/gnss_mi355x.h
--- a/include/gnss_mi355x.h
+++ b/include/gnss_mi355x.h
@@ -156,8 +156,12 @@
 #define GNSS_OPT_VT_BLOCKS    9
 #define GNSS_OPT_FORCE_PEER   10
 #define GNSS_OPT_VT_SPAN      11
-#define GNSS_OPT_COUNT        12
+#define GNSS_OPT_SLOT_PATH    12
+#define GNSS_OPT_COUNT        13
 int  gnss_ctx_set_option(gnss_ctx *ctx, int key, int64_t value);
+int  gnss_lane_boundaries(const double *taps, const double *post, int n_taps, int lane_samples,
+                          double cps_max);
+int  gnss_ctx_lane_path(const gnss_ctx *ctx);
 
 int  gnss_dev_alloc(gnss_ctx *ctx, uint64_t nbytes, void **dev_ptr);
 int  gnss_dev_free(gnss_ctx *ctx, void *dev_ptr);
```

New measurement: 400,900 (median of 6 runs). 1.03x the previous value.
